# starreeze/drin

Measured on AMD Instinct MI355X. Metric: mention x candidate pairs scored/sec, higher is better.
Workload: dtype bf16x3; 1 GPU; wikimel-shaped scoring forward: 100-cand (+1 answer slot), D=768, R=2048, L=128, P=49, T=64 token-level entity text; parallelism=dp1 (mentions sharded, no collective)

## Files before the change

### drin_amd/csrc/fused.h

```cpp
#pragma once
#include <hip/hip_runtime.h>
#include <stddef.h>
#include <stdint.h>
#include <string.h>

#include "../../include/drin_hip.h"
#include "layout.h"

namespace drin {

struct Prepared {
  size_t wcat1, bcat1, ecat, etmp, k_t, k_i, c_txt, c_img, cb_t, cb_i, total;
  size_t p_ctxt, p_cimg, p_wh2;
  size_t p_wmt, p_wmi, p_wcat1, p_ecat, p_wet, p_wei, p_wh1;
  size_t p_cimg_f16;
  size_t cimg_f16_scale;
  void build(const drin_config& c) {
    const size_t D = c.embed_dim, R = c.image_dim;
    size_t off = 0;
    auto take = [&off](size_t n) {
      const size_t o = off;
      off += (n + 63) & ~(size_t)63;
      return o;
    };
    wcat1 = take(2 * D * D);
    bcat1 = take(2 * D);
    ecat = take(D * (D + R));
    etmp = take(D * (D + R));
    k_t = take(D);
    k_i = take(D);
    c_txt = take(D * D);
    c_img = take(D * R);
    cb_t = take(D);
    cb_i = take(D);
    p_ctxt = take(D * D);
    p_cimg = take(D * R);
    p_wh2 = take(D * D);
    p_wmt = take(D * D);
    p_wmi = take(D * R);
    p_wcat1 = take(2 * D * D);
    p_ecat = take(D * (D + R));
    p_wet = take(D * D);
    p_wei = take(D * R);
    p_wh1 = take(D * D);
    p_cimg_f16 = take(D * R / 2 + 2);
    cimg_f16_scale = take(2);
    total = off;
  }
};

int fused_supported(const drin_config* c);
int cached_chunks_per_mention(const drin_config& c);

struct StreamArgs {
  const void* entity_text;
  const int64_t* entity_mask;
  const void* entity_image;
  const void* entity_object;
  const float* entity_object_score;
  const int64_t* entity_index;
  int64_t num_entities;
  int32_t* index_status;
  const float* miet;
  const float* mtei;
  const float* span_mean;
  const void* mobj;
  const float* mscore;
  const float* fu;
  const float* q;
  const float* k_t;
  const float* k_i;
  float* xt_out;
  void* xt_hi;
  void* xt_lo;
  void* xi_hi;
  void* xi_lo;
  float* xi_scale;
  void* xi_f16;
  float* e0m;
  float* e1m;
  float* s_part;
  float* s_text;
  float* s_img;
  float* sig;
  int B, N, D4, R4, T, Km, Ke, chunks, ldq, ldfu, dynamic, bf16_features;
  int act_e;
  float mask[4];
  float cos_eps, miei_eps, clip;
};

struct PairArgs {
  const float* h_text;
  const float* h_image;
  const float* hm;
  const float* c_t;
  const float* c_i;
  const float* gamma;
  const float* beta;
  const float* e0m;
  const float* e1m;
  float* et1;
  void* et1_hi;
  void* et1_lo;
  float* s2_part;
  int B, N, D4, chunks, ldhm;
  int act_v;
  float ln_eps;
};

struct FinalArgs {
  const float* h2;
  const float* hm2;
  const float* b_h2;
  const float* gamma;
  const float* beta;
  const float* e1m;
  const float* mt2;
  float* scores;
  int B, N, D4, chunks;
  int act_v;
  float ln_eps, cos_eps;
};

template <class Args>
Args shaped_args(const drin_config& c) {
  Args a;
  memset(&a, 0, sizeof(a));
  a.B = c.batch, a.N = c.num_candidates, a.D4 = c.embed_dim / 4;
  return a;
}
template <class Args>
void set_vertex_fields(Args& a, const drin_config& c) {
  a.ln_eps = c.layer_norm_eps, a.act_v = vertex_act(&c);
}
template <class Args>
void set_edge_fields(Args& a, const drin_config& c) {
  a.R4 = c.image_dim / 4;
  a.Km = c.mention_objects;
  a.dynamic = c.dynamic_edges != 0;
  a.act_e = edge_act(&c);
  for (int k = 0; k < 4; ++k) a.mask[k] = c.edge_enabled[k];
  a.cos_eps = c.cosine_eps, a.miei_eps = c.miei_eps, a.clip = c.clip_scale;
}

size_t entity_stream_lds_bytes(const StreamArgs& a);
int launch_entity_stream(const StreamArgs& a, hipStream_t st);
int launch_reduce_stream_partials(const float* part, float* s_text, float* s_img, float* sig, int B, int D, int R,
                                  int chunks, hipStream_t st);
int launch_mention_input1(const float* T, const float* T2, const float* sig, const float* b_et, const float* b_ei,
                          const float* v0, float* out, int B, int D, int N, hipStream_t st);
int launch_pair_layer1(const PairArgs& a, hipStream_t st);
int launch_mention_input2(const float* part, const float* mt1, float* out, int B, int D, int N, int chunks,
                          hipStream_t st);
int launch_pair_final(const FinalArgs& a, hipStream_t st);

struct GemmScratch {
  float* p = nullptr;
  size_t floats = 0;
};
int run_folded_head(const drin_config* cfg, const drin_batch* b, const drin_params* params, const float* prepared, const Prepared& P,
                    bool weight_planes, float* span_mean, float* mimg, float* vm0, float* hmfu, GemmScratch mention_sk, hipStream_t st);
int run_folded_mention_finish(const drin_config* cfg, const drin_params* params, const float* prepared, const Prepared& P,
                              bool weight_planes, float* vm1, float* hm2, GemmScratch mention_sk, hipStream_t st);
int run_folded_tail(const drin_config* cfg, const drin_params* params, const float* prepared, const Prepared& P, int chunks,
                    const float* s2_part, const float* vm1, float* agg2, float* mt2, const float* hm2, const float* e1m, float* h2,
                    const float* et1, const void* et1_hi, bool weight_planes, GemmScratch mention_sk, GemmScratch pair_sk,
                    float* scores, hipStream_t st);
}
```

### drin_amd/csrc/fused_forward.hip

```cpp
#include <string.h>

#include "fused.h"
#include "internal.h"
#include "layout.h"

namespace drin {

constexpr int kMixedMinCandidates = 64;

struct FusedLayout {
  size_t span_mean, mimg, vm0, hmfu, q, e0m, e1m, xt, s_part, s_text, s_img, sig, tm, tm2, agg1, vm1, hm2, h_text, h_image,
      et1, s2_part, agg2, mt2, p_xt, p_xi, p_et1, xi_scale, splitk, splitk_floats, pair_splitk, pair_splitk_floats, total;
  int chunks;
  void build(const drin_config& c) {
    const size_t B = c.batch, N = c.num_candidates, D = c.embed_dim, R = c.image_dim, M = B * N;
    chunks = (int)(B >= 2048 ? (N + 127) / 128 : B >= 1024 ? (N + 47) / 48 : (N + 15) / 16);
    size_t off = 0;
    auto take = [&off](size_t n) {
      const size_t o = off;
      off += (n + 63) & ~(size_t)63;
      return o;
    };
    span_mean = take(B * D);
    mimg = take(B * R);
    vm0 = take(2 * B * D);
    hmfu = take(2 * B * 2 * D);
    q = take(2 * B * (D + R));
    e0m = take(4 * M);
    e1m = take(4 * M);
    xt = take(c.entity_tokens > 0 ? M * D : 0);
    s_part = take(B * chunks * (2 * D + 2 * R + 4));
    s_text = take(2 * B * D);
    s_img = take(2 * B * R);
    sig = take(4 * B);
    tm = take(2 * B * D);
    tm2 = take(2 * B * D);
    agg1 = take(2 * B * D);
    vm1 = take(2 * B * D);
    hm2 = take(2 * B * D);
    h_text = take(M * D);
    h_image = take(M * D);
    et1 = take(M * D);
    s2_part = take(B * chunks * 2 * D);
    agg2 = take(B * D);
    mt2 = take(B * D);
    const bool planes = c.precision == DRIN_PREC_BF16X3 || c.precision == DRIN_PREC_BF16X3_ALL || c.precision == DRIN_PREC_BF16X3_IF16;
    p_xt = take(planes ? M * D : 0);
    p_xi = take(!planes ? 0 : c.num_entities > 0 ? M * R : c.precision == DRIN_PREC_BF16X3_IF16 ? M * R / 2 : 0);
    p_et1 = take(planes ? M * D : 0);
    xi_scale = take(c.precision == DRIN_PREC_BF16X3_IF16 ? M : 0);
    splitk_floats = 2 * B <= 512 ? 8 * 2 * B * (D + R) : 0;
    if (planes && splitk_floats < (size_t)192 * 65536) splitk_floats = (size_t)192 * 65536;
    splitk = take(splitk_floats);
    pair_splitk_floats = 0;
    {
      const size_t tiles = ((M + 255) / 256) * ((D + 255) / 256);
      if (planes && tiles <= 128)
        for (size_t s : {16, 8, 6, 4, 3, 2})
          if (tiles * s <= 256) {
            pair_splitk_floats = s * ((M + 255) / 256 * 256) * D;
            break;
          }
    }
    pair_splitk = take(pair_splitk_floats);
    total = off;
  }
};

static bool if16_gate(const drin_config* c, bool indexed) {
  const int64_t M = (int64_t)c->batch * c->num_candidates;
  return c->precision == DRIN_PREC_BF16X3_IF16 && !indexed && c->feature_dtype == DRIN_FEAT_F32 &&
         c->num_candidates >= kMixedMinCandidates && c->embed_dim == 768 && c->image_dim == 2048 &&
         cdiv(M, 256) * cdiv(c->embed_dim, 256) >= 128;
}

#ifndef DRIN_SIDE_WGS
#define DRIN_SIDE_WGS 64
#endif
#ifndef DRIN_SIDE_PERMILLE
#define DRIN_SIDE_PERMILLE 900
#endif
#ifndef DRIN_SIDE_MIN_TILES
#define DRIN_SIDE_MIN_TILES 1200
#endif
constexpr int kSideWgs = DRIN_SIDE_WGS;
constexpr int kSidePermille = DRIN_SIDE_PERMILLE;
constexpr int64_t kSideMinTiles = DRIN_SIDE_MIN_TILES;
#ifdef DRIN_SIDE_PROBE
static int g_probe_wgs = kSideWgs, g_probe_permille = kSidePermille;
extern "C" __attribute__((visibility("default"))) void drin_probe_side_plan(int wgs, int permille) { g_probe_wgs = wgs, g_probe_permille = permille; }
#endif
struct SidePlan {
  int64_t S = 0;
  int G = 0;
};
static SidePlan image_side_plan(const drin_config* c, bool indexed, bool capturing) {
  SidePlan plan;
  int wgs = kSideWgs, permille = kSidePermille;
#ifdef DRIN_SIDE_PROBE
  wgs = g_probe_wgs, permille = g_probe_permille;
#endif
  const bool split = c->precision == DRIN_PREC_BF16X3 || c->precision == DRIN_PREC_BF16X3_ALL || c->precision == DRIN_PREC_BF16X3_IF16;
  if (capturing || indexed || !split || if16_gate(c, indexed) || wgs <= 0 || permille <= 0) return plan;
  const int D = c->embed_dim, R = c->image_dim;
  if ((D % 32) || (R % 32) || c->batch <= 0) return plan;
  const int64_t M = (int64_t)c->batch * c->num_candidates;
  const int64_t nx = cdiv(D, 256), row_tiles = cdiv(M, 256), tiles = row_tiles * nx;
  if (tiles < 192 || tiles < kSideMinTiles || tiles > ((int64_t)1 << 28)) return plan;
  FusedLayout L;
  L.build(*c);
  const int64_t whole_rows = gemm_p4_whole_tiles(tiles, R, L.splitk_floats > 0, L.splitk_floats) / nx;
  int64_t S = (row_tiles * permille + 500) / 1000;
  S = S < whole_rows ? S : whole_rows;
  S = S < row_tiles - 1 ? S : row_tiles - 1;
  if (S <= 0) return plan;
  plan.S = S;
  plan.G = (int)(wgs < S * nx ? wgs : S * nx);
  return plan;
}

struct SideJoin {
  SideLane* lane = nullptr;
  hipStream_t st = nullptr;
  int join() {
    if (!lane) return DRIN_OK;
    const hipError_t e = hipStreamWaitEvent(st, lane->join, 0);
    lane = nullptr;
    return e == hipSuccess ? DRIN_OK : hip_fail(e, "hipStreamWaitEvent(side stream)");
  }
  ~SideJoin() { (void)join(); }
};

int fused_supported(const drin_config* c) {
  if (c->num_layers != 2) {
    set_error("fused path: built for num_layers == 2 (got %d); use drin_forward", c->num_layers);
    return DRIN_E_UNSUPPORTED;
  }
  if (c->vector_edges) {
    set_error("fused path: vector edge features (model.py:112-116) run on the layer-by-layer path; use drin_forward");
    return DRIN_E_UNSUPPORTED;
  }
  if (c->mention_object_inner > 1 || c->entity_object_inner > 1 || c->entity_image_inner > 1) {
    set_error("fused path: inner feature dims > 1 need the pooled path of drin_forward");
    return DRIN_E_UNSUPPORTED;
  }
  const bool tiny = c->embed_dim <= 256 && c->image_dim <= 256;
  const bool full = c->embed_dim <= 768 && c->image_dim <= 2048;
  if (!tiny && !full) {
    set_error("fused path: D=%d R=%d outside the built instantiations", c->embed_dim, c->image_dim);
    return DRIN_E_UNSUPPORTED;
  }
  return DRIN_OK;
}

}

using namespace drin;

extern "C" {

int drin_split_planes(const float* x, void* hi, void* lo, int64_t n, void* stream) {
  DRIN_BIND_DEVICE(stream, x, "drin_split_planes");
  if (!x || !hi || !lo) {
    set_error("drin_split_planes: NULL argument");
    return DRIN_E_NULL;
  }
  return launch_split_planes(x, hi, lo, n, (hipStream_t)stream);
}

int drin_linear_planes_fwd(const void* x_hi, const void* x_lo, const void* w_hi, const void* w_lo, const float* bias,
                           float* y, int64_t rows, int32_t n_out, int32_t k, void* stream) {
  DRIN_BIND_DEVICE(stream, y, "drin_linear_planes_fwd");
  if (!x_hi || !w_hi || !w_lo || !y) {
    set_error("drin_linear_planes_fwd: NULL argument");
    return DRIN_E_NULL;
  }
  return launch_gemm_x3_planes(x_hi, x_lo, k, w_hi, w_lo, k, bias, y, n_out, rows, n_out, k, (hipStream_t)stream);
}

int drin_fused_supported(const drin_config* cfg) {
  DRIN_TRY(validate_config(cfg));
  return fused_supported(cfg);
}

size_t drin_prepared_bytes(const drin_config* cfg) {
  if (validate_config(cfg) != DRIN_OK || fused_supported(cfg) != DRIN_OK) return 0;
  Prepared P;
  P.build(*cfg);
  return P.total * sizeof(float);
}

int drin_prepare(const drin_config* cfg, const drin_params* params, void* prepared, size_t prepared_bytes,
                 void* stream) {
  DRIN_BIND_DEVICE(stream, prepared, "drin_prepare");
  RoctxRange range("drin_prepare");
  DRIN_TRY(validate_config(cfg));
  DRIN_TRY(fused_supported(cfg));
  if (!params || !prepared) {
    set_error("drin_prepare: NULL argument");
    return DRIN_E_NULL;
  }
  Prepared P;
  P.build(*cfg);
  if (prepared_bytes < P.total * sizeof(float) || !aligned16(prepared)) {
    set_error("drin_prepare: buffer has %zu bytes (needs %zu) or is not 16-byte aligned", prepared_bytes,
              P.total * sizeof(float));
    return DRIN_E_WORKSPACE;
  }
  hipStream_t st = (hipStream_t)stream;
  float* pb = (float*)prepared;
  const int D = cfg->embed_dim, R = cfg->image_dim;
  const drin_layer_params& L1 = params->layer[0];
  const int F32 = DRIN_PREC_F32;
  auto copy = [&](float* dst, const float* src, size_t n) -> int {
    hipError_t e = hipMemcpyAsync(dst, src, n * sizeof(float), hipMemcpyDeviceToDevice, st);
    return e == hipSuccess ? DRIN_OK : hip_fail(e, "hipMemcpyAsync(prepare)");
  };
  DRIN_TRY(copy(pb + P.wcat1, L1.w_h, (size_t)D * D));
  DRIN_TRY(copy(pb + P.wcat1 + (size_t)D * D, L1.w_u, (size_t)D * D));
  {
    hipError_t e = hipMemsetAsync(pb + P.bcat1, 0, D * sizeof(float), st);
    if (e != hipSuccess) return hip_fail(e, "hipMemsetAsync(prepare)");
  }
  DRIN_TRY(copy(pb + P.bcat1 + D, L1.b_u, D));
  DRIN_TRY(launch_gemm_nn(L1.w_v, D, params->w_entity_text, D, pb + P.etmp, D + R, D, D, D, false, F32, st));
  DRIN_TRY(launch_gemm_nn(L1.w_v, D, params->w_entity_image, R, pb + P.etmp + D, D + R, D, R, D, false, F32, st));
  DRIN_TRY(launch_transpose(pb + P.etmp, pb + P.ecat, D, D + R, st));
  DRIN_TRY(launch_gemm_nt(params->b_entity_text, D, L1.w_v, D, L1.b_v, pb + P.k_t, D, 1, D, D, false, F32, st));
  DRIN_TRY(launch_gemm_nt(params->b_entity_image, D, L1.w_v, D, L1.b_v, pb + P.k_i, D, 1, D, D, false, F32, st));
  DRIN_TRY(launch_gemm_nn(L1.w_h, D, params->w_entity_text, D, pb + P.c_txt, D, D, D, D, false, F32, st));
  DRIN_TRY(launch_gemm_nn(L1.w_h, D, params->w_entity_image, R, pb + P.c_img, R, D, R, D, false, F32, st));
  DRIN_TRY(launch_gemm_nt(params->b_entity_text, D, L1.w_h, D, L1.b_h, pb + P.cb_t, D, 1, D, D, false, F32, st));
  DRIN_TRY(launch_gemm_nt(params->b_entity_image, D, L1.w_h, D, L1.b_h, pb + P.cb_i, D, 1, D, D, false, F32, st));
  {
    const size_t dd = (size_t)D * D, dr = (size_t)D * R;
    __bf16* q = reinterpret_cast<__bf16*>(pb + P.p_ctxt);
    DRIN_TRY(launch_split_planes(pb + P.c_txt, q, q + dd, dd, st));
    q = reinterpret_cast<__bf16*>(pb + P.p_cimg);
    DRIN_TRY(launch_split_planes(pb + P.c_img, q, q + dr, dr, st));
    DRIN_TRY(launch_to_f16_scaled(pb + P.c_img, pb + P.p_cimg_f16, (int64_t)dr, pb + P.cimg_f16_scale, st));
    q = reinterpret_cast<__bf16*>(pb + P.p_wh2);
    DRIN_TRY(launch_split_planes(params->layer[1].w_h, q, q + dd, dd, st));
    struct { size_t off; const float* w; size_t n; } extra[] = {
        {P.p_wmt, params->w_mention_text, dd},  {P.p_wmi, params->w_mention_image, dr},
        {P.p_wcat1, pb + P.wcat1, 2 * dd},      {P.p_ecat, pb + P.ecat, dd + dr},
        {P.p_wet, params->w_entity_text, dd},   {P.p_wei, params->w_entity_image, dr},
        {P.p_wh1, L1.w_h, dd}};
    for (const auto& e : extra) {
      q = reinterpret_cast<__bf16*>(pb + e.off);
      DRIN_TRY(launch_split_planes(e.w, q, q + e.n, e.n, st));
    }
  }
  return DRIN_OK;
}

}

namespace drin {

static int folded_precision(const drin_config* c) { return c->precision == DRIN_PREC_BF16X3_IF16 ? (int)DRIN_PREC_BF16X3 : c->precision; }

int run_folded_head(const drin_config* cfg, const drin_batch* b, const drin_params* params, const float* pb, const Prepared& P,
                    bool weight_planes, float* span_mean, float* mimg, float* vm0, float* hmfu, GemmScratch sk, hipStream_t st) {
  const int B = cfg->batch, D = cfg->embed_dim, R = cfg->image_dim, prec = folded_precision(cfg);
  auto wp = [&](size_t plane_off) -> const float* { return weight_planes ? pb + plane_off : nullptr; };
  if (cfg->feature_dtype == DRIN_FEAT_BF16) {
    DRIN_TRY(launch_span_mean_bf16(b->mention_text, b->mention_start, b->mention_end, span_mean, B, cfg->mention_tokens, D, st));
    DRIN_TRY(launch_axis_mean_bf16(b->mention_image, mimg, B, cfg->image_regions, R, st));
  } else {
    DRIN_TRY(launch_span_mean(b->mention_text, b->mention_start, b->mention_end, span_mean, B, cfg->mention_tokens, D, st));
    DRIN_TRY(launch_axis_mean(b->mention_image, mimg, B, cfg->image_regions, R, st));
  }
  DRIN_TRY(launch_gemm_nt_pair({span_mean, params->w_mention_text, params->b_mention_text, vm0, D, D, D, B, D, D, wp(P.p_wmt)},
                               {mimg, params->w_mention_image, params->b_mention_image, vm0 + (size_t)B * D, R, R, D, B, D, R, wp(P.p_wmi)},
                               prec, st, sk.p, sk.floats));
  return launch_gemm_nt(vm0, D, pb + P.wcat1, D, pb + P.bcat1, hmfu, 2 * D, 2 * (int64_t)B, 2 * D, D, false, prec, st, sk.p, sk.floats,
                        wp(P.p_wcat1));
}

int run_folded_mention_finish(const drin_config* cfg, const drin_params* params, const float* pb, const Prepared& P,
                              bool weight_planes, float* vm1, float* hm2, GemmScratch sk, hipStream_t st) {
  const int B = cfg->batch, D = cfg->embed_dim;
  const drin_layer_params& L1 = params->layer[0];
  DRIN_TRY(launch_layernorm_gelu(vm1, L1.ln_weight, L1.ln_bias, vm1, nullptr, nullptr, 2 * (int64_t)B, D, cfg->layer_norm_eps, st,
                                 vertex_act(cfg)));
  return launch_gemm_nt(vm1, D, params->layer[1].w_h, D, nullptr, hm2, D, 2 * (int64_t)B, D, D, false, folded_precision(cfg), st, sk.p,
                        sk.floats, weight_planes ? pb + P.p_wh2 : nullptr);
}

int run_folded_tail(const drin_config* cfg, const drin_params* params, const float* pb, const Prepared& P, int chunks,
                    const float* s2_part, const float* vm1, float* agg2, float* mt2, const float* hm2, const float* e1m, float* h2,
                    const float* et1, const void* et1_hi, bool weight_planes, GemmScratch sk, GemmScratch pair_sk, float* scores,
                    hipStream_t st) {
  const int B = cfg->batch, N = cfg->num_candidates, D = cfg->embed_dim, prec = folded_precision(cfg);
  const int64_t M = (int64_t)B * N;
  const drin_layer_params& L2 = params->layer[1];
  DRIN_TRY(launch_mention_input2(s2_part, vm1, agg2, B, D, N, chunks, st));
  DRIN_TRY(launch_gemm_nt(agg2, D, L2.w_h, D, L2.b_h, mt2, D, B, D, D, false, prec, st, sk.p, sk.floats,
                          weight_planes ? pb + P.p_wh2 : nullptr));
  DRIN_TRY(launch_layernorm_gelu(mt2, L2.ln_weight, L2.ln_bias, mt2, nullptr, nullptr, B, D, cfg->layer_norm_eps, st, vertex_act(cfg)));
  if (et1_hi) {
    const __bf16* e1 = static_cast<const __bf16*>(et1_hi);
    const __bf16* w2 = reinterpret_cast<const __bf16*>(pb + P.p_wh2);
    DRIN_TRY(launch_gemm_x3_planes(e1, e1 + (size_t)M * D, D, w2, w2 + (size_t)D * D, D, nullptr, h2, D, M, D, D, st, pair_sk.p,
                                   pair_sk.floats));
  } else {
    DRIN_TRY(launch_gemm_nt(et1, D, L2.w_h, D, nullptr, h2, D, M, D, D, false, prec, st));
  }
  FinalArgs fa = shaped_args<FinalArgs>(*cfg);
  set_vertex_fields(fa, *cfg);
  fa.h2 = h2;
  fa.hm2 = hm2;
  fa.b_h2 = L2.b_h;
  fa.gamma = L2.ln_weight;
  fa.beta = L2.ln_bias;
  fa.e1m = e1m;
  fa.mt2 = mt2;
  fa.scores = scores;
  fa.chunks = chunks;
  fa.cos_eps = cfg->cosine_eps;
  return launch_pair_final(fa, st);
}

static int forward_prepared_on_stream(const drin_config* cfg, const drin_batch* b, const drin_params* params, const void* prepared,
                                      void* workspace, float* scores, hipStream_t st) {
  FusedLayout L;
  L.build(*cfg);
  Prepared P;
  P.build(*cfg);
  float* ws = (float*)workspace;
  const float* pb = (const float*)prepared;
  const int B = cfg->batch, N = cfg->num_candidates, D = cfg->embed_dim, R = cfg->image_dim;
  const int64_t M = (int64_t)B * N;
  if (B == 0) return DRIN_OK;
  const int prec = folded_precision(cfg);
  const bool dyn = cfg->dynamic_edges != 0;
  const bool tokens = cfg->entity_tokens > 0;
  const bool planes = (prec == DRIN_PREC_BF16X3 || prec == DRIN_PREC_BF16X3_ALL) && (D % 32 == 0) && (R % 32 == 0);
  const bool indexed = b->entity_index != nullptr;
  const bool xi_planes = planes && indexed;
  const bool if16 = if16_gate(cfg, indexed) && gemm_f16_planes_fits(ws + L.p_xi, R, pb + P.p_cimg_f16, R, ws + L.h_image, D, M, D, R);
  hipStreamCaptureStatus capture = hipStreamCaptureStatusNone;
  if (hipStreamIsCapturing(st, &capture) != hipSuccess) {
    (void)hipGetLastError();
    capture = hipStreamCaptureStatusActive;
  }
  SidePlan side = image_side_plan(cfg, indexed, capture != hipStreamCaptureStatusNone);
  if (!aligned16(b->entity_image) || !aligned16(ws + L.h_image) || !b->entity_image) side = SidePlan();
  if (b->entity_text_cls) {
    set_error("drin_forward_prepared: entity_text_cls (text pooled ahead of time) is a form of the training entry points");
    return DRIN_E_UNSUPPORTED;
  }
  if (indexed && cfg->num_entities <= 0) {
    set_error("drin_forward_prepared: entity_index given but cfg.num_entities = %d", cfg->num_entities);
    return DRIN_E_SHAPE;
  }
  if (indexed && !planes) {
    set_error("drin_forward_prepared: entity_index needs the split-bf16 precision (the stream kernel gathers the "
              "GEMM operands as planes); gather on the caller side for DRIN_PREC_F32");
    return DRIN_E_UNSUPPORTED;
  }
  const bool bf16_feat = cfg->feature_dtype == DRIN_FEAT_BF16;
  if (bf16_feat && !planes) {
    set_error("drin_forward_prepared: bf16 features need the split-bf16 precision (DRIN_PREC_BF16X3) and D, R multiples of 32");
    return DRIN_E_UNSUPPORTED;
  }
  __bf16* xt_hi = reinterpret_cast<__bf16*>(ws + L.p_xt);
  __bf16* xi_hi = reinterpret_cast<__bf16*>(ws + L.p_xi);
  __bf16* e1_hi = reinterpret_cast<__bf16*>(ws + L.p_et1);
  const size_t MD = (size_t)M * D, MR = (size_t)M * R;
  const drin_layer_params& L1 = params->layer[0];

  auto wp = [&](size_t plane_off) -> const float* { return planes ? pb + plane_off : nullptr; };
  const GemmScratch msk{L.splitk_floats ? ws + L.splitk : nullptr, L.splitk_floats};
  float* vm0 = ws + L.vm0;
  float* hmfu = ws + L.hmfu;
  const bool xt_exact = bf16_feat && !tokens;
  const GemmScratch psk = L.pair_splitk_floats ? GemmScratch{ws + L.pair_splitk, L.pair_splitk_floats} : msk;
  auto image_rows_product = [&](hipStream_t on, RowTiles rows) -> int {
    const __bf16* ci = reinterpret_cast<const __bf16*>(pb + P.p_cimg);
    if (bf16_feat)
      return launch_gemm_x3_planes(b->entity_image, nullptr, R, ci, ci + (size_t)D * R, R, nullptr, ws + L.h_image, D, M, D, R, on, psk.p,
                                   psk.floats, rows);
    return launch_gemm_nt_bf16x3_p4((const float*)b->entity_image, R, ci, ci + (size_t)D * R, R, nullptr, ws + L.h_image, D, M, D, R, on, false,
                                    aligned16(psk.p) ? psk.p : nullptr, psk.floats, rows);
  };
  SideJoin side_join;
  if (side.S > 0) {
    SideLane* lane = nullptr;
    DRIN_TRY(side_lane(&lane));
    std::lock_guard<std::mutex> order(lane->order);
    hipError_t e = hipEventRecord(lane->fork, st);
    if (e == hipSuccess) e = hipStreamWaitEvent(lane->stream, lane->fork, 0);
    if (e != hipSuccess) return hip_fail(e, "fork to the side stream");
    const int rc = image_rows_product(lane->stream, RowTiles{0, side.S, side.G});
    e = hipEventRecord(lane->join, lane->stream);
    side_join.lane = lane, side_join.st = st;
    if (rc != DRIN_OK) return rc;
    if (e != hipSuccess) return hip_fail(e, "hipEventRecord(side stream)");
  }
  DRIN_TRY(run_folded_head(cfg, b, params, pb, P, planes, ws + L.span_mean, ws + L.mimg, vm0, hmfu, msk, st));
  if (dyn)
    DRIN_TRY(launch_gemm_nt(hmfu + D, 2 * D, pb + P.ecat, D, nullptr, ws + L.q, D + R, 2 * (int64_t)B, D + R, D, false, prec, st, msk.p,
                            msk.floats, wp(P.p_ecat)));
  StreamArgs sa = shaped_args<StreamArgs>(*cfg);
  set_edge_fields(sa, *cfg);
  sa.entity_text = b->entity_text;
  sa.entity_mask = b->entity_text_mask;
  sa.entity_image = b->entity_image;
  sa.entity_object = b->entity_object;
  sa.entity_object_score = b->entity_object_score;
  sa.entity_index = b->entity_index;
  sa.num_entities = cfg->num_entities;
  sa.index_status = b->index_status;
  sa.miet = b->miet_similarity;
  sa.mtei = b->mtei_similarity;
  sa.span_mean = ws + L.span_mean;
  sa.mobj = b->mention_object;
  sa.mscore = b->mention_object_score;
  sa.fu = hmfu + D;
  sa.ldfu = 2 * D;
  sa.q = ws + L.q;
  sa.ldq = D + R;
  sa.k_t = pb + P.k_t;
  sa.k_i = pb + P.k_i;
  sa.xt_out = planes ? nullptr : ws + L.xt;
  if (planes) {
    sa.xt_hi = xt_hi;
    sa.xt_lo = xt_exact ? nullptr : xt_hi + MD;
    if (xi_planes) {
      sa.xi_hi = xi_hi;
      sa.xi_lo = bf16_feat ? nullptr : xi_hi + MR;
    }
  }
  sa.xi_scale = if16 ? ws + L.xi_scale : nullptr;
  sa.xi_f16 = if16 ? static_cast<void*>(xi_hi) : nullptr;
  sa.e0m = ws + L.e0m;
  sa.e1m = ws + L.e1m;
  sa.s_part = ws + L.s_part;
  sa.T = cfg->entity_tokens;
  sa.Ke = cfg->entity_objects;
  sa.chunks = L.chunks;
  sa.bf16_features = bf16_feat ? 1 : 0;
  sa.s_text = ws + L.s_text;
  sa.s_img = ws + L.s_img;
  sa.sig = ws + L.sig;
  DRIN_TRY(launch_entity_stream(sa, st));
  if (L.chunks > 1)
    DRIN_TRY(launch_reduce_stream_partials(ws + L.s_part, ws + L.s_text, ws + L.s_img, ws + L.sig, B, D, R, L.chunks, st));
  DRIN_TRY(launch_gemm_nt_pair({ws + L.s_text, params->w_entity_text, nullptr, ws + L.tm, D, D, D, 2 * (int64_t)B, D, D, wp(P.p_wet)},
                               {ws + L.s_img, params->w_entity_image, nullptr, ws + L.tm2, R, R, D, 2 * (int64_t)B, D, R,
                                wp(P.p_wei)},
                               prec, st, msk.p, msk.floats));
  DRIN_TRY(launch_mention_input1(ws + L.tm, ws + L.tm2, ws + L.sig, params->b_entity_text, params->b_entity_image, vm0, ws + L.agg1, B, D, N, st));
  float* vm1 = ws + L.vm1;
  DRIN_TRY(launch_gemm_nt(ws + L.agg1, D, L1.w_h, D, L1.b_h, vm1, D, 2 * (int64_t)B, D, D, false, prec, st, msk.p, msk.floats, wp(P.p_wh1)));
  DRIN_TRY(run_folded_mention_finish(cfg, params, pb, P, planes, vm1, ws + L.hm2, msk, st));
  if (planes) {
    const __bf16* ct = reinterpret_cast<const __bf16*>(pb + P.p_ctxt);
    const __bf16* ci = reinterpret_cast<const __bf16*>(pb + P.p_cimg);
    DRIN_TRY(launch_gemm_x3_planes(xt_hi, xt_exact ? nullptr : xt_hi + MD, D, ct, ct + (size_t)D * D, D, nullptr, ws + L.h_text, D, M, D,
                                   D, st, psk.p, psk.floats));
    if (if16)
      DRIN_TRY(launch_gemm_f16_planes(xi_hi, R, pb + P.p_cimg_f16, R, ws + L.xi_scale, pb + P.cimg_f16_scale, ws + L.h_image, D, M, D, R,
                                      st, psk.p, psk.floats));
    else if (xi_planes)
      DRIN_TRY(launch_gemm_x3_planes(xi_hi, bf16_feat ? nullptr : xi_hi + MR, R, ci, ci + (size_t)D * R, R, nullptr, ws + L.h_image, D, M,
                                     D, R, st, psk.p, psk.floats));
    else if (side.S > 0) {
      DRIN_TRY(side_join.join());
      DRIN_TRY(image_rows_product(st, RowTiles{side.S, -1, 0}));
    } else if (bf16_feat)
      DRIN_TRY(launch_gemm_x3_planes(b->entity_image, nullptr, R, ci, ci + (size_t)D * R, R, nullptr, ws + L.h_image, D, M, D, R, st, psk.p,
                                     psk.floats));
    else
      DRIN_TRY(launch_gemm_nt_bf16x3(b->entity_image, R, pb + P.c_img, R, nullptr, ws + L.h_image, D, M, D, R, st, ci, ci + (size_t)D * R,
                                     false, psk.p, psk.floats));
  } else {
    const float* x_t = tokens ? ws + L.xt : b->entity_text;
    DRIN_TRY(launch_gemm_nt(x_t, D, pb + P.c_txt, D, nullptr, ws + L.h_text, D, M, D, D, false, prec, st));
    DRIN_TRY(launch_gemm_nt(b->entity_image, R, pb + P.c_img, R, nullptr, ws + L.h_image, D, M, D, R, false, prec, st));
  }
  PairArgs pa = shaped_args<PairArgs>(*cfg);
  set_vertex_fields(pa, *cfg);
  pa.h_text = ws + L.h_text;
  pa.h_image = ws + L.h_image;
  pa.hm = hmfu;
  pa.ldhm = 2 * D;
  pa.c_t = pb + P.cb_t;
  pa.c_i = pb + P.cb_i;
  pa.gamma = L1.ln_weight;
  pa.beta = L1.ln_bias;
  pa.e0m = ws + L.e0m;
  pa.e1m = ws + L.e1m;
  pa.et1 = planes ? nullptr : ws + L.et1;
  if (planes) {
    pa.et1_hi = e1_hi;
    pa.et1_lo = e1_hi + MD;
  }
  pa.s2_part = ws + L.s2_part;
  pa.chunks = L.chunks;
  DRIN_TRY(launch_pair_layer1(pa, st));
  return run_folded_tail(cfg, params, pb, P, L.chunks, ws + L.s2_part, vm1, ws + L.agg2, ws + L.mt2, ws + L.hm2, ws + L.e1m, ws + L.h_text,
                         planes ? nullptr : ws + L.et1, planes ? e1_hi : nullptr, planes, msk, psk, scores, st);
}

}

extern "C" {

int32_t drin_workgroups_per_mention(const drin_config* cfg, int32_t cached) {
  if (validate_config(cfg) != DRIN_OK || fused_supported(cfg) != DRIN_OK) return 0;
  if (cached) return cached_chunks_per_mention(*cfg);
  FusedLayout L;
  L.build(*cfg);
  return L.chunks;
}

int32_t drin_image_contraction_side_tiles(const drin_config* cfg, int32_t indexed) {
  if (validate_config(cfg) != DRIN_OK || fused_supported(cfg) != DRIN_OK) return 0;
  return (int32_t)image_side_plan(cfg, indexed != 0, false).S;
}

int32_t drin_image_contraction_passes(const drin_config* cfg, int32_t indexed) {
  if (validate_config(cfg) != DRIN_OK || fused_supported(cfg) != DRIN_OK) return 0;
  if (cfg->precision == DRIN_PREC_F32) return 0;
  if (if16_gate(cfg, indexed != 0)) return 1;
  return cfg->feature_dtype == DRIN_FEAT_BF16 ? 2 : 3;
}

int drin_index_status(int32_t* index_status, void* stream) {
  if (!index_status) {
    set_error("drin_index_status: NULL argument");
    return DRIN_E_NULL;
  }
  DRIN_BIND_DEVICE(stream, index_status, "drin_index_status");
  int32_t w[4] = {0, 0, 0, 0};
  hipError_t e = hipMemcpyAsync(w, index_status, sizeof(w), hipMemcpyDeviceToHost, (hipStream_t)stream);
  if (e == hipSuccess) e = hipStreamSynchronize((hipStream_t)stream);
  if (e != hipSuccess) return hip_fail(e, "drin_index_status");
  if (w[0] == 0) return DRIN_OK;
  e = hipMemsetAsync(index_status, 0, sizeof(w), (hipStream_t)stream);
  if (e != hipSuccess) return hip_fail(e, "drin_index_status(reset)");
  const long long value = (long long)(((uint64_t)(uint32_t)w[3] << 32) | (uint32_t)w[2]);
  set_error("entity_index out of range: candidate row %lld at pair %d (b * N + n) is outside the entity tables - the row was clamped "
            "and a WRONG entity scored; drin/data.py:87-93 raises IndexError here", value, (int)w[1]);
  return DRIN_E_INDEX;
}

size_t drin_fused_workspace_bytes(const drin_config* cfg) {
  if (validate_config(cfg) != DRIN_OK || fused_supported(cfg) != DRIN_OK) return 0;
  FusedLayout L;
  L.build(*cfg);
  return L.total * sizeof(float);
}

int drin_forward_prepared(const drin_config* cfg, const drin_batch* b, const drin_params* params, const void* prepared,
                          void* workspace, size_t workspace_bytes, float* scores, void* stream) {
  DRIN_BIND_DEVICE(stream, workspace, "drin_forward_prepared");
  RoctxRange range("drin_forward_prepared");
  DRIN_TRY(validate_config(cfg));
  DRIN_TRY(fused_supported(cfg));
  if (!b || !params || !prepared || !workspace || !scores) {
    set_error("drin_forward_prepared: NULL argument");
    return DRIN_E_NULL;
  }
  FusedLayout L;
  L.build(*cfg);
  if (workspace_bytes < L.total * sizeof(float) || !aligned16(workspace)) {
    set_error("drin_forward_prepared: workspace has %zu bytes (needs %zu) or is not 16-byte aligned", workspace_bytes,
              L.total * sizeof(float));
    return DRIN_E_WORKSPACE;
  }
  return forward_prepared_on_stream(cfg, b, params, prepared, workspace, scores, (hipStream_t)stream);
}

}
```

### drin_amd/csrc/fused_kernels.hip

```cpp
#include "device_utils.h"
#include "fused.h"
#include "internal.h"
#include "row_ops.h"

namespace drin {

template <int DV, int RV, bool TOKENS, bool EXACT, typename FT, bool XSCALE = false>
__global__ void __launch_bounds__(256, 2) k_entity_stream(const StreamArgs a) {
  extern __shared__ __attribute__((aligned(16))) float lds[];
  const FT* const f_text = static_cast<const FT*>(a.entity_text);
  const FT* const f_image = static_cast<const FT*>(a.entity_image);
  const FT* const f_object = static_cast<const FT*>(a.entity_object);
  const FT* const f_mobj = static_cast<const FT*>(a.mobj);
  const int D4 = EXACT ? DV * 64 : a.D4, R4 = EXACT ? RV * 64 : a.R4, D = D4 * 4, R = R4 * 4;
  constexpr bool RP = sizeof(FT) == 2 && (RV % 2) == 0;
  auto load_r = [&](const FT* row) -> Row<RV> {
    if constexpr (RP)
      return load_row_stream_pair<RV>(row, (int)(threadIdx.x & 63), R4);
    else
      return load_row_stream<RV>(row, (int)(threadIdx.x & 63), R4);
  };
  float* l_mobj = lds;
  float* l_q = l_mobj + a.Km * R;
  float* l_red = l_q + 2 * R;
  float* l_mt = l_red + 2 * D + 2 * R;
  float* l_small = l_mt + 3 * D;
  const int wave = threadIdx.x >> 6, lane = threadIdx.x & 63;
  const int64_t b = blockIdx.y;
  const int per = (a.N + a.chunks - 1) / a.chunks;
  const int n_begin = blockIdx.x * per, n_end = min(a.N, n_begin + per);
  const bool dyn = a.dynamic != 0;

  for (int i = threadIdx.x; i < a.Km * R4; i += 256) st4(l_mobj + i * 4, ld4(f_mobj + (b * a.Km) * R + i * 4));
  for (int i = threadIdx.x; i < D4; i += 256) st4(l_mt + i * 4, ld4(a.span_mean + b * D + i * 4));
  if (dyn) {
    for (int i = threadIdx.x; i < 2 * R4; i += 256) {
      const int which = i / R4, c4 = i - which * R4;
      st4(l_q + i * 4, ld4(a.q + ((int64_t)which * a.B + b) * a.ldq + D + c4 * 4));
    }
    for (int i = threadIdx.x; i < 2 * D4; i += 256) {
      const int which = i / D4, c4 = i - which * D4;
      st4(l_mt + D + i * 4, ld4(a.q + ((int64_t)which * a.B + b) * a.ldq + c4 * 4));
    }
  }
  __syncthreads();
  for (int i = wave; i < a.Km; i += 4) {
    float s = 0.f;
    for (int c4 = lane; c4 < R4; c4 += 64) {
      const float4 v = ld4(l_mobj + i * R + c4 * 4);
      s += dot4(v, v);
    }
    s = wave_sum(s);
    if (lane == 0) l_small[i] = fmaxf(sqrtf(s), a.cos_eps);
  }
  float m_t_norm;
  {
    const Row<DV> m_t = load_row<DV>(l_mt, lane, D4);
    m_t_norm = fmaxf(sqrtf(wave_sum(dot_rows<DV>(m_t, m_t))), a.cos_eps);
  }
  float kap_tt = 0.f, kap_ti = 0.f, kap_it = 0.f, kap_ii = 0.f;
  if (dyn) {
    const Row<DV> fu_t = load_row<DV>(a.fu + b * a.ldfu, lane, D4);
    const Row<DV> fu_i = load_row<DV>(a.fu + ((int64_t)a.B + b) * a.ldfu, lane, D4);
    const Row<DV> k_t = load_row<DV>(a.k_t, lane, D4), k_i = load_row<DV>(a.k_i, lane, D4);
    kap_tt = wave_sum(dot_rows<DV>(fu_t, k_t));
    kap_ti = wave_sum(dot_rows<DV>(fu_t, k_i));
    kap_it = wave_sum(dot_rows<DV>(fu_i, k_t));
    kap_ii = wave_sum(dot_rows<DV>(fu_i, k_i));
  }
  __syncthreads();

  Row<DV> S_tt = zero_row<DV>(), S_it = zero_row<DV>();
  Row<RV> S_ti = zero_row<RV>(), S_ii = zero_row<RV>();
  float sg_tt = 0.f, sg_ti = 0.f, sg_it = 0.f, sg_ii = 0.f;
  const float inv_d = 1.0f / (float)D;

  for (int n = n_begin + wave; n < n_end; n += 4) {
    const int64_t p = b * a.N + n;
    int64_t e = p;
    if (a.entity_index) {
      const int64_t raw = a.entity_index[p];
      e = raw < 0 ? 0 : (raw >= a.num_entities ? a.num_entities - 1 : raw);
      if (e != raw && lane == 0) report_bad_index(a.index_status, p, raw);
    }
    Row<DV> xt;
    float tt;
    if (TOKENS) {
      const int T = a.T;
      int cnt = 0;
      for (int t = lane; t < T; t += 64) cnt += (int)a.entity_mask[e * T + t];
      cnt = (int)wave_sum((float)cnt);
      int stop = cnt - 1;
      if (stop < 0) stop += T;
      stop = stop < 0 ? 0 : (stop > T ? T : stop);
      const FT* base = f_text + e * (int64_t)T * D;
      constexpr bool FLAT = sizeof(FT) == 2 && EXACT && DV == 3;
      const Row<DV> cls = load_row_stream<DV>(base, lane, D4);
      Row<DV> acc = zero_row<DV>();
      int t = 1;
      if constexpr (FLAT) {
        float f0[8], f1[8], f2[8];
#pragma unroll
        for (int i = 0; i < 8; ++i) f0[i] = f1[i] = f2[i] = 0.f;
        const char* flat = reinterpret_cast<const char*>(base) + (size_t)lane * 16;
        auto add8 = [](float (&f)[8], const u32x4_t v) {
#pragma unroll
          for (int i = 0; i < 4; ++i) {
            f[2 * i] += __builtin_bit_cast(float, v[i] << 16);
            f[2 * i + 1] += __builtin_bit_cast(float, v[i] & 0xffff0000u);
          }
        };
        for (; t + 8 <= stop; t += 8) {
          u32x4_t r[4][3];
#pragma unroll
          for (int u = 0; u < 4; ++u)
#pragma unroll
            for (int k = 0; k < 3; ++k) r[u][k] = ld16_stream(flat + (size_t)(t + 2 * u) * (2 * 768) + k * 1024);
#pragma unroll
          for (int u = 0; u < 4; ++u) {
            add8(f0, r[u][0]);
            add8(f1, r[u][1]);
            add8(f2, r[u][2]);
          }
        }
        for (; t + 2 <= stop; t += 2) {
          const u32x4_t r0 = ld16_stream(flat + (size_t)t * (2 * 768)), r1 = ld16_stream(flat + (size_t)t * (2 * 768) + 1024),
                        r2 = ld16_stream(flat + (size_t)t * (2 * 768) + 2048);
          add8(f0, r0);
          add8(f1, r1);
          add8(f2, r2);
        }
        float* scr = l_red + wave * 768;
#pragma unroll
        for (int i = 0; i < 8; ++i) {
          const float y1 = __shfl_xor(f1[i], 32), y2 = __shfl_xor(f2[i], 32);
          f0[i] += lane < 32 ? y1 : y2;
          f1[i] += y2;
        }
        st4(scr + 8 * lane, make_float4(f0[0], f0[1], f0[2], f0[3]));
        st4(scr + 8 * lane + 4, make_float4(f0[4], f0[5], f0[6], f0[7]));
        if (lane < 32) {
          st4(scr + 512 + 8 * lane, make_float4(f1[0], f1[1], f1[2], f1[3]));
          st4(scr + 512 + 8 * lane + 4, make_float4(f1[4], f1[5], f1[6], f1[7]));
        }
        __builtin_amdgcn_wave_barrier();
#pragma unroll
        for (int j = 0; j < DV; ++j) acc.v[j] = ld4(scr + 4 * (lane + 64 * j));
        __builtin_amdgcn_wave_barrier();
      } else if constexpr (sizeof(FT) == 2 && (EXACT || DV == 1)) {
        for (; t + 8 <= stop; t += 8) {
          Row<DV> r[8];
#pragma unroll
          for (int u = 0; u < 8; ++u) r[u] = load_row_stream<DV>(base + (int64_t)(t + u) * D, lane, D4);
#pragma unroll
          for (int u = 0; u < 8; ++u)
#pragma unroll
            for (int j = 0; j < DV; ++j) acc.v[j] = acc.v[j] + r[u].v[j];
        }
      }
      for (; t + 4 <= stop; t += 4) {
        const Row<DV> r0 = load_row_stream<DV>(base + (int64_t)t * D, lane, D4);
        const Row<DV> r1 = load_row_stream<DV>(base + (int64_t)(t + 1) * D, lane, D4);
        const Row<DV> r2 = load_row_stream<DV>(base + (int64_t)(t + 2) * D, lane, D4);
        const Row<DV> r3 = load_row_stream<DV>(base + (int64_t)(t + 3) * D, lane, D4);
#pragma unroll
        for (int j = 0; j < DV; ++j) acc.v[j] = (((acc.v[j] + r0.v[j]) + r1.v[j]) + r2.v[j]) + r3.v[j];
      }
      for (; t < stop; ++t) {
        const Row<DV> r0 = load_row_stream<DV>(base + (int64_t)t * D, lane, D4);
#pragma unroll
        for (int j = 0; j < DV; ++j) acc.v[j] = acc.v[j] + r0.v[j];
      }
      const float den = stop > 1 ? (float)(stop - 1) : 0.0f;
#pragma unroll
      for (int j = 0; j < DV; ++j)
        xt.v[j] = make_float4(acc.v[j].x / den, acc.v[j].y / den, acc.v[j].z / den, acc.v[j].w / den);
      if (a.xt_out) store_row<DV>(a.xt_out + p * D, xt, lane, D4);
      const float xy = wave_sum(dot_row_lds<DV>(cls, l_mt, lane, D4)), yy = wave_sum(dot_rows<DV>(cls, cls));
      tt = xy / (m_t_norm * fmaxf(sqrtf(yy), a.cos_eps));
    } else {
      xt = load_row_stream<DV>(f_text + e * D, lane, D4);
      const float xy = wave_sum(dot_row_lds<DV>(xt, l_mt, lane, D4)), yy = wave_sum(dot_rows<DV>(xt, xt));
      tt = xy / (m_t_norm * fmaxf(sqrtf(yy), a.cos_eps));
    }
    if (a.xt_hi) store_row_planes<DV>(a.xt_hi, a.xt_lo, p * D, xt, lane, D4);
    float sim = 0.f, wsum = 0.f;
    for (int j = 0; j < a.Ke; ++j) {
      const Row<RV> eo = load_r(f_object + (e * a.Ke + j) * R);
      const float ny = fmaxf(sqrtf(wave_sum(dot_rows<RV>(eo, eo))), a.cos_eps);
      const float es = a.entity_object_score[e * a.Ke + j];
      for (int i = 0; i < a.Km; ++i) {
        const float xy = wave_sum(dot_row_lds<RV, RP>(eo, l_mobj + i * R, lane, R4));
        const float w = a.mscore[b * a.Km + i] * es;
        sim += xy / (l_small[i] * ny) * w;
        wsum += w;
      }
    }
    const float ii = sim / (wsum + a.miei_eps);
    const Row<RV> xi = load_r(f_image + e * R);
    if (a.xi_hi) store_row_planes<RV, RP>(a.xi_hi, a.xi_lo, p * R, xi, lane, R4);
    if constexpr (XSCALE) {
      float m = 0.f;
#pragma unroll
      for (int j = 0; j < RV; ++j) m = fmaxf(m, fmaxf(fmaxf(fabsf(xi.v[j].x), fabsf(xi.v[j].y)), fmaxf(fabsf(xi.v[j].z), fabsf(xi.v[j].w))));
      const float sc = cache_field_scale(wave_max(m));
      if (lane == 0) a.xi_scale[p] = sc;
      store_row_f16_scaled<RV, RP>(a.xi_f16, p * R, xi, 1.0f / sc, lane);
    }
    const float e_tt = tt * a.mask[0];
    const float e_ti = (a.mtei[p] / a.clip) * a.mask[1];
    const float e_it = (a.miet[p] / a.clip) * a.mask[2];
    const float e_ii = ii * a.mask[3];
    float n_tt = e_tt, n_ti = e_ti, n_it = e_it, n_ii = e_ii;
    if (dyn) {
      const float d_tt = wave_sum(dot_row_lds<DV>(xt, l_mt + D, lane, D4));
      const float d_it = wave_sum(dot_row_lds<DV>(xt, l_mt + 2 * D, lane, D4));
      const float d_ti = wave_sum(dot_row_lds<RV, RP>(xi, l_q, lane, R4));
      const float d_ii = wave_sum(dot_row_lds<RV, RP>(xi, l_q + R, lane, R4));
      n_tt = edge_act_apply(a.act_e, (d_tt + kap_tt) * inv_d + e_tt);
      n_ti = edge_act_apply(a.act_e, (d_ti + kap_ti) * inv_d + e_ti);
      n_it = edge_act_apply(a.act_e, (d_it + kap_it) * inv_d + e_it);
      n_ii = edge_act_apply(a.act_e, (d_ii + kap_ii) * inv_d + e_ii);
    }
    if (lane == 0) {
      const int64_t M = (int64_t)a.B * a.N;
      a.e0m[p] = e_tt;
      a.e0m[M + p] = e_ti;
      a.e0m[2 * M + p] = e_it;
      a.e0m[3 * M + p] = e_ii;
      a.e1m[p] = n_tt * a.mask[0];
      a.e1m[M + p] = n_ti * a.mask[1];
      a.e1m[2 * M + p] = n_it * a.mask[2];
      a.e1m[3 * M + p] = n_ii * a.mask[3];
    }
    axpy_row<DV>(S_tt, e_tt, xt);
    axpy_row<DV>(S_it, e_it, xt);
    axpy_row<RV>(S_ti, e_ti, xi);
    axpy_row<RV>(S_ii, e_ii, xi);
    sg_tt += e_tt;
    sg_ti += e_ti;
    sg_it += e_it;
    sg_ii += e_ii;
  }

  for (int w = 0; w < 4; ++w) {
    __syncthreads();
    if (wave == w) {
#pragma unroll
      for (int j = 0; j < DV; ++j) {
        const int c4 = lane + 64 * j;
        if (c4 < D4) {
          float* p0 = l_red + c4 * 4;
          float* p1 = l_red + D + c4 * 4;
          st4(p0, w == 0 ? S_tt.v[j] : ld4(p0) + S_tt.v[j]);
          st4(p1, w == 0 ? S_it.v[j] : ld4(p1) + S_it.v[j]);
        }
      }
#pragma unroll
      for (int j = 0; j < RV; ++j) {
        const int c4 = row_col4<RP>(lane, j);
        if (c4 < R4) {
          float* p0 = l_red + 2 * D + c4 * 4;
          float* p1 = l_red + 2 * D + R + c4 * 4;
          st4(p0, w == 0 ? S_ti.v[j] : ld4(p0) + S_ti.v[j]);
          st4(p1, w == 0 ? S_ii.v[j] : ld4(p1) + S_ii.v[j]);
        }
      }
      if (lane == 0) {
        float* s4 = l_small + a.Km;
        s4[0] = (w == 0 ? 0.f : s4[0]) + sg_tt;
        s4[1] = (w == 0 ? 0.f : s4[1]) + sg_ti;
        s4[2] = (w == 0 ? 0.f : s4[2]) + sg_it;
        s4[3] = (w == 0 ? 0.f : s4[3]) + sg_ii;
      }
    }
  }
  __syncthreads();
  if (a.chunks == 1) {
    for (int i = threadIdx.x; i < 2 * D4; i += 256) {
      const int which = i / D4, c4 = i - which * D4;
      st4(a.s_text + ((int64_t)which * a.B + b) * D + c4 * 4, ld4(l_red + i * 4));
    }
    for (int i = threadIdx.x; i < 2 * R4; i += 256) {
      const int which = i / R4, c4 = i - which * R4;
      st4(a.s_img + ((int64_t)which * a.B + b) * R + c4 * 4, ld4(l_red + 2 * D + i * 4));
    }
    if (threadIdx.x < 4) a.sig[(int64_t)threadIdx.x * a.B + b] = l_small[a.Km + threadIdx.x];
    return;
  }
  float* out = a.s_part + (b * a.chunks + blockIdx.x) * (int64_t)(2 * D + 2 * R + 4);
  for (int i = threadIdx.x; i < (2 * D + 2 * R) / 4; i += 256) st4(out + i * 4, ld4(l_red + i * 4));
  if (threadIdx.x < 4) out[2 * D + 2 * R + threadIdx.x] = l_small[a.Km + threadIdx.x];
}

size_t entity_stream_lds_bytes(const StreamArgs& a) {
  const size_t D = (size_t)a.D4 * 4, R = (size_t)a.R4 * 4;
  return sizeof(float) * (a.Km * R + 2 * R + 2 * D + 2 * R + 3 * D + a.Km + 4);
}

template <int DV, int RV, bool TOKENS, bool EXACT, typename FT, bool XSCALE = false>
static int launch_stream_ft(const StreamArgs& a, hipStream_t st) {
  const size_t lds = entity_stream_lds_bytes(a);
  auto kern = k_entity_stream<DV, RV, TOKENS, EXACT, FT, XSCALE>;
  static DynLdsOptIn opt_in;
  if (lds > 48 * 1024)
    DRIN_TRY(ensure_dynamic_lds(opt_in, reinterpret_cast<const void*>(kern), (int)lds, "hipFuncSetAttribute(entity_stream)"));
  KernelTimer timer(DRIN_KC_STREAM, st);
  hipLaunchKernelGGL(kern, dim3((unsigned)a.chunks, (unsigned)a.B), dim3(256), lds, st, a);
  DRIN_CHECK_LAUNCH("k_entity_stream");
  return DRIN_OK;
}

template <int DV, int RV, bool TOKENS, bool EXACT>
static int launch_stream_t(const StreamArgs& a, hipStream_t st) {
  if (a.xi_scale != nullptr) {
    if constexpr (EXACT && DV == 3) {
      if (a.xi_f16 == nullptr) {
        set_error("entity_stream: xi_scale without xi_f16");
        return DRIN_E_NULL;
      }
      if (!a.bf16_features) return launch_stream_ft<DV, RV, TOKENS, EXACT, float, true>(a, st);
    }
    set_error("entity_stream: the scaled fp16 image plane is built for fp32-stored rows at D = 768, R = 2048");
    return DRIN_E_UNSUPPORTED;
  }
  return a.bf16_features ? launch_stream_ft<DV, RV, TOKENS, EXACT, __bf16>(a, st)
                         : launch_stream_ft<DV, RV, TOKENS, EXACT, float>(a, st);
}

int launch_entity_stream(const StreamArgs& a, hipStream_t st) {
  if (a.B <= 0) return DRIN_OK;
  if (a.B > 65535) {
    set_error("entity_stream: batch %d exceeds the grid limit; split the batch", a.B);
    return DRIN_E_SHAPE;
  }
  const bool tok = a.T > 0;
  if (a.D4 <= 64 && a.R4 <= 64)
    return tok ? launch_stream_t<1, 1, true, false>(a, st) : launch_stream_t<1, 1, false, false>(a, st);
  if (a.D4 == 192 && a.R4 == 512)
    return tok ? launch_stream_t<3, 8, true, true>(a, st) : launch_stream_t<3, 8, false, true>(a, st);
  if (a.D4 <= 192 && a.R4 <= 512)
    return tok ? launch_stream_t<3, 8, true, false>(a, st) : launch_stream_t<3, 8, false, false>(a, st);
  set_error("entity_stream: D=%d R=%d outside the built instantiations", a.D4 * 4, a.R4 * 4);
  return DRIN_E_UNSUPPORTED;
}

__global__ void __launch_bounds__(256) k_reduce_stream_partials(const float* __restrict__ part, float* __restrict__ s_text,
                                                                float* __restrict__ s_img, float* __restrict__ sig,
                                                                int B, int D, int R, int chunks) {
  const int64_t b = blockIdx.y;
  const int width = 2 * D + 2 * R + 4;
  const int i = (blockIdx.x * 256 + threadIdx.x) * 4;
  if (i >= width) return;
  const float* src = part + (b * chunks) * (int64_t)width + i;
  float4 s = make_float4(0.f, 0.f, 0.f, 0.f);
  int c = 0;
  for (; c + 4 <= chunks; c += 4) {
    const float4 v0 = ld4(src + (int64_t)c * width), v1 = ld4(src + (int64_t)(c + 1) * width);
    const float4 v2 = ld4(src + (int64_t)(c + 2) * width), v3 = ld4(src + (int64_t)(c + 3) * width);
    s = (((s + v0) + v1) + v2) + v3;
  }
  for (; c < chunks; ++c) s = s + ld4(src + (int64_t)c * width);
  if (i < D) {
    st4(s_text + b * D + i, s);
  } else if (i < 2 * D) {
    st4(s_text + ((int64_t)B + b) * D + (i - D), s);
  } else if (i < 2 * D + R) {
    st4(s_img + b * R + (i - 2 * D), s);
  } else if (i < 2 * D + 2 * R) {
    st4(s_img + ((int64_t)B + b) * R + (i - 2 * D - R), s);
  } else {
    sig[b] = s.x;
    sig[(int64_t)B + b] = s.y;
    sig[2 * (int64_t)B + b] = s.z;
    sig[3 * (int64_t)B + b] = s.w;
  }
}

int launch_reduce_stream_partials(const float* part, float* s_text, float* s_img, float* sig, int B, int D, int R,
                                  int chunks, hipStream_t st) {
  if (B <= 0) return DRIN_OK;
  KernelTimer timer(DRIN_KC_GCN, st);
  hipLaunchKernelGGL(k_reduce_stream_partials, dim3((unsigned)cdiv((2 * D + 2 * R + 4) / 4, 256), (unsigned)B), dim3(256), 0,
                     st, part, s_text, s_img, sig, B, D, R, chunks);
  DRIN_CHECK_LAUNCH("k_reduce_stream_partials");
  return DRIN_OK;
}

__global__ void __launch_bounds__(256) k_mention_input1(const float* __restrict__ T, const float* __restrict__ T2,
                                                        const float* __restrict__ sig,
                                                        const float* __restrict__ b_et, const float* __restrict__ b_ei,
                                                        const float* __restrict__ v0, float* __restrict__ out, int B,
                                                        int D, float inv_n) {
  const int64_t i = (int64_t)blockIdx.x * 256 + threadIdx.x;
  if (i >= 2 * (int64_t)B * D) return;
  const int d = (int)(i % D);
  const int64_t row = i / D;
  const int t = (int)(row / B);
  const int64_t b = row - (int64_t)t * B;
  const float sa = sig[(int64_t)(t == 0 ? 0 : 2) * B + b], sb = sig[(int64_t)(t == 0 ? 1 : 3) * B + b];
  out[i] = ((T[i] + T2[i]) + sa * b_et[d] + sb * b_ei[d]) * inv_n + v0[i];
}

int launch_mention_input1(const float* T, const float* T2, const float* sig, const float* b_et, const float* b_ei,
                          const float* v0, float* out, int B, int D, int N, hipStream_t st) {
  if (B <= 0) return DRIN_OK;
  KernelTimer timer(DRIN_KC_GCN, st);
  hipLaunchKernelGGL(k_mention_input1, dim3((unsigned)cdiv(2 * (int64_t)B * D, 256)), dim3(256), 0, st, T, T2, sig,
                     b_et, b_ei, v0, out, B, D, 1.0f / (float)N);
  DRIN_CHECK_LAUNCH("k_mention_input1");
  return DRIN_OK;
}

__global__ void __launch_bounds__(256) k_transpose(const float* __restrict__ in, float* __restrict__ out, int rows,
                                                   int cols) {
  __shared__ float tile[32][33];
  const int tx = threadIdx.x & 31, ty = threadIdx.x >> 5;
  const int r0 = blockIdx.y * 32, c0 = blockIdx.x * 32;
  for (int i = ty; i < 32; i += 8)
    if (r0 + i < rows && c0 + tx < cols) tile[i][tx] = in[(int64_t)(r0 + i) * cols + c0 + tx];
  __syncthreads();
  for (int i = ty; i < 32; i += 8)
    if (c0 + i < cols && r0 + tx < rows) out[(int64_t)(c0 + i) * rows + r0 + tx] = tile[tx][i];
}

int launch_transpose(const float* in, float* out, int rows, int cols, hipStream_t st) {
  if (rows <= 0 || cols <= 0) return DRIN_OK;
  KernelTimer timer(DRIN_KC_GCN, st);
  hipLaunchKernelGGL(k_transpose, dim3((unsigned)cdiv(cols, 32), (unsigned)cdiv(rows, 32)), dim3(256), 0, st, in, out,
                     rows, cols);
  DRIN_CHECK_LAUNCH("k_transpose");
  return DRIN_OK;
}

template <int DV, bool EXACT, bool GENERIC_ACT = false>
__global__ void __launch_bounds__(256) k_pair_layer1(const PairArgs a) {
  __shared__ __attribute__((aligned(16))) float l_red[2 * DV * 256];
  __shared__ __attribute__((aligned(16))) float l_const[6 * DV * 256];
  const int D4 = EXACT ? DV * 64 : a.D4, D = D4 * 4;
  const int wave = threadIdx.x >> 6, lane = threadIdx.x & 63;
  const int64_t b = blockIdx.y;
  const int64_t M = (int64_t)a.B * a.N;
  const int per = (a.N + a.chunks - 1) / a.chunks;
  const int n_begin = blockIdx.x * per, n_end = min(a.N, n_begin + per);
  constexpr int LD = DV * 256;
  {
    const float* src[6] = {a.hm + b * a.ldhm, a.hm + ((int64_t)a.B + b) * a.ldhm, a.c_t, a.c_i, a.gamma, a.beta};
#pragma unroll
    for (int v = 0; v < 6; ++v)
      for (int i = threadIdx.x; i < D4; i += 256) st4(l_const + v * LD + i * 4, ld4(src[v] + i * 4));
  }
  __syncthreads();
  const float *l_hm_t = l_const, *l_hm_i = l_const + LD, *l_ct = l_const + 2 * LD, *l_ci = l_const + 3 * LD;
  const float *l_gamma = l_const + 4 * LD, *l_beta = l_const + 5 * LD;
  Row<DV> S_t = zero_row<DV>(), S_i = zero_row<DV>();
  for (int n = n_begin + wave; n < n_end; n += 4) {
    const int64_t p = b * a.N + n;
    const Row<DV> ht = load_row_stream<DV>(a.h_text + p * D, lane, D4);
    const Row<DV> hi = load_row_stream<DV>(a.h_image + p * D, lane, D4);
    const float e_tt = a.e0m[p], e_ti = a.e0m[M + p], e_it = a.e0m[2 * M + p], e_ii = a.e0m[3 * M + p];
    const Row<DV> et1 = ln_gelu_row_lds<DV, GENERIC_ACT>(combine_rows_lds<DV>(ht, e_tt, l_hm_t, e_it, l_hm_i, l_ct, lane, D4),
                                                         l_gamma, l_beta, lane, D4, a.ln_eps, a.act_v);
    if (a.et1) store_row<DV>(a.et1 + p * D, et1, lane, D4);
    if (a.et1_hi) store_row_planes<DV>(a.et1_hi, a.et1_lo, p * D, et1, lane, D4);
    axpy_row_pk<DV>(S_t, a.e1m[p], et1);
    const Row<DV> ei1 = ln_gelu_row_lds<DV, GENERIC_ACT>(combine_rows_lds<DV>(hi, e_ti, l_hm_t, e_ii, l_hm_i, l_ci, lane, D4),
                                                         l_gamma, l_beta, lane, D4, a.ln_eps, a.act_v);
    axpy_row_pk<DV>(S_i, a.e1m[M + p], ei1);
  }
  for (int w = 0; w < 4; ++w) {
    __syncthreads();
    if (wave == w) {
#pragma unroll
      for (int j = 0; j < DV; ++j) {
        float* p0 = l_red + (j * 64 + lane) * 4;
        float* p1 = l_red + DV * 256 + (j * 64 + lane) * 4;
        st4(p0, w == 0 ? S_t.v[j] : ld4(p0) + S_t.v[j]);
        st4(p1, w == 0 ? S_i.v[j] : ld4(p1) + S_i.v[j]);
      }
    }
  }
  __syncthreads();
  float* out = a.s2_part + (b * a.chunks + blockIdx.x) * (int64_t)(2 * D);
  for (int i = threadIdx.x; i < 2 * D4; i += 256) {
    const int which = i / D4, c4 = i - which * D4;
    st4(out + which * D + c4 * 4, ld4(l_red + which * DV * 256 + c4 * 4));
  }
}

int launch_pair_layer1(const PairArgs& a, hipStream_t st) {
  if (a.B <= 0) return DRIN_OK;
  KernelTimer timer(DRIN_KC_GCN, st);
  if (a.act_v != DRIN_ACT_GELU && a.D4 <= 64)
    hipLaunchKernelGGL((k_pair_layer1<1, false, true>), dim3((unsigned)a.chunks, (unsigned)a.B), dim3(256), 0, st, a);
  else if (a.act_v != DRIN_ACT_GELU && a.D4 <= 192)
    hipLaunchKernelGGL((k_pair_layer1<3, false, true>), dim3((unsigned)a.chunks, (unsigned)a.B), dim3(256), 0, st, a);
  else if (a.D4 <= 64)
    hipLaunchKernelGGL((k_pair_layer1<1, false>), dim3((unsigned)a.chunks, (unsigned)a.B), dim3(256), 0, st, a);
  else if (a.D4 == 192)
    hipLaunchKernelGGL((k_pair_layer1<3, true>), dim3((unsigned)a.chunks, (unsigned)a.B), dim3(256), 0, st, a);
  else if (a.D4 < 192)
    hipLaunchKernelGGL((k_pair_layer1<3, false>), dim3((unsigned)a.chunks, (unsigned)a.B), dim3(256), 0, st, a);
  else {
    set_error("pair_layer1: D=%d outside the built instantiations", a.D4 * 4);
    return DRIN_E_UNSUPPORTED;
  }
  DRIN_CHECK_LAUNCH("k_pair_layer1");
  return DRIN_OK;
}

__global__ void __launch_bounds__(256) k_mention_input2(const float* __restrict__ part, const float* __restrict__ mt1,
                                                        float* __restrict__ out, int D, int chunks, float inv_n) {
  const int64_t b = blockIdx.y;
  const int d = blockIdx.x * 256 + threadIdx.x;
  if (d >= D) return;
  float st = 0.f, si = 0.f;
  for (int c = 0; c < chunks; ++c) {
    const float* p = part + (b * chunks + c) * (int64_t)(2 * D);
    st += p[d];
    si += p[D + d];
  }
  out[b * D + d] = (st * inv_n + si * inv_n) + mt1[b * D + d];
}

int launch_mention_input2(const float* part, const float* mt1, float* out, int B, int D, int N, int chunks,
                          hipStream_t st) {
  if (B <= 0) return DRIN_OK;
  KernelTimer timer(DRIN_KC_GCN, st);
  hipLaunchKernelGGL(k_mention_input2, dim3((unsigned)cdiv(D, 256), (unsigned)B), dim3(256), 0, st, part, mt1, out, D,
                     chunks, 1.0f / (float)N);
  DRIN_CHECK_LAUNCH("k_mention_input2");
  return DRIN_OK;
}

template <int DV, bool EXACT, bool GENERIC_ACT = false>
__global__ void __launch_bounds__(256) k_pair_final(const FinalArgs a) {
  __shared__ __attribute__((aligned(16))) float l_const[6 * DV * 256];
  const int D4 = EXACT ? DV * 64 : a.D4, D = D4 * 4;
  const int wave = threadIdx.x >> 6, lane = threadIdx.x & 63;
  const int64_t b = blockIdx.y;
  const int64_t M = (int64_t)a.B * a.N;
  const int per = (a.N + a.chunks - 1) / a.chunks;
  const int n_begin = blockIdx.x * per, n_end = min(a.N, n_begin + per);
  constexpr int LD = DV * 256;
  {
    const float* src[6] = {a.hm2 + b * D, a.hm2 + ((int64_t)a.B + b) * D, a.b_h2, a.gamma, a.beta, a.mt2 + b * D};
#pragma unroll
    for (int v = 0; v < 6; ++v)
      for (int i = threadIdx.x; i < D4; i += 256) st4(l_const + v * LD + i * 4, ld4(src[v] + i * 4));
  }
  __syncthreads();
  const Row<DV> mt2 = load_row<DV>(l_const + 5 * LD, lane, D4);
  const float xx = wave_sum(dot_rows<DV>(mt2, mt2));
  for (int n = n_begin + wave; n < n_end; n += 4) {
    const int64_t p = b * a.N + n;
    const Row<DV> h = load_row_stream<DV>(a.h2 + p * D, lane, D4);
    const Row<DV> et2 = ln_gelu_row_lds<DV, GENERIC_ACT>(
        combine_rows_lds<DV>(h, a.e1m[p], l_const, a.e1m[2 * M + p], l_const + LD, l_const + 2 * LD, lane, D4),
        l_const + 3 * LD, l_const + 4 * LD, lane, D4, a.ln_eps, a.act_v);
    const float xy = wave_sum(dot_rows_pk<DV>(mt2, et2));
    const float yy = wave_sum(dot_rows_pk<DV>(et2, et2));
    if (lane == 0) a.scores[p] = cosine_from_sums(xy, xx, yy, a.cos_eps);
  }
}

int launch_pair_final(const FinalArgs& a, hipStream_t st) {
  if (a.B <= 0) return DRIN_OK;
  KernelTimer timer(DRIN_KC_GCN, st);
  if (a.act_v != DRIN_ACT_GELU && a.D4 <= 64)
    hipLaunchKernelGGL((k_pair_final<1, false, true>), dim3((unsigned)a.chunks, (unsigned)a.B), dim3(256), 0, st, a);
  else if (a.act_v != DRIN_ACT_GELU && a.D4 <= 192)
    hipLaunchKernelGGL((k_pair_final<3, false, true>), dim3((unsigned)a.chunks, (unsigned)a.B), dim3(256), 0, st, a);
  else if (a.D4 <= 64)
    hipLaunchKernelGGL((k_pair_final<1, false>), dim3((unsigned)a.chunks, (unsigned)a.B), dim3(256), 0, st, a);
  else if (a.D4 == 192)
    hipLaunchKernelGGL((k_pair_final<3, true>), dim3((unsigned)a.chunks, (unsigned)a.B), dim3(256), 0, st, a);
  else if (a.D4 < 192)
    hipLaunchKernelGGL((k_pair_final<3, false>), dim3((unsigned)a.chunks, (unsigned)a.B), dim3(256), 0, st, a);
  else {
    set_error("pair_final: D=%d outside the built instantiations", a.D4 * 4);
    return DRIN_E_UNSUPPORTED;
  }
  DRIN_CHECK_LAUNCH("k_pair_final");
  return DRIN_OK;
}

}
```

Baseline: 28.34 million pairs/s.

## Fold mention layer-1 aggregation into pair kernel using precomputed h_text/h_image sums

Rather than have the entity stream kernel accumulate edge-weighted entity text/image sums and then run two GEMMs (through the entity projections and layer-1 weights), the pair layer-1 kernel now accumulates edge-weighted sums of the already-projected h_text/h_image rows plus edge-weight totals. A new small kernel combines them with precomputed bias-projected vectors to produce vm1 directly. This drops the large image-dim reductions from the stream kernel, two GEMMs, and several weight plane copies, and shrinks stream LDS use. It also raises occupancy bounds on the stream and pair kernels, widens the stream unroll, disables the side-GEMM overlap when LDS allows co-residency, and tweaks the side permille. The pair kernel takes on more register and LDS pressure, and the IF16 path still needs an image-sum reduction and GEMM.

```diff
diff --git a/drin_amd/csrc/fused.h b/drin_amd/csrc/fused.h
--- a/drin_amd/csrc/fused.h
+++ b/drin_amd/csrc/fused.h
@@ -10,9 +10,9 @@
 namespace drin {
 
 struct Prepared {
-  size_t wcat1, bcat1, ecat, etmp, k_t, k_i, c_txt, c_img, cb_t, cb_i, total;
+  size_t wcat1, bcat1, ecat, etmp, k_t, k_i, c_txt, c_img, cb_t, cb_i, hb_t, hb_i, total;
   size_t p_ctxt, p_cimg, p_wh2;
-  size_t p_wmt, p_wmi, p_wcat1, p_ecat, p_wet, p_wei, p_wh1;
+  size_t p_wmt, p_wmi, p_wcat1, p_ecat;
   size_t p_cimg_f16;
   size_t cimg_f16_scale;
   void build(const drin_config& c) {
@@ -40,11 +40,10 @@
     p_wmi = take(D * R);
     p_wcat1 = take(2 * D * D);
     p_ecat = take(D * (D + R));
-    p_wet = take(D * D);
-    p_wei = take(D * R);
-    p_wh1 = take(D * D);
     p_cimg_f16 = take(D * R / 2 + 2);
     cimg_f16_scale = take(2);
+    hb_t = take(D);
+    hb_i = take(D);
     total = off;
   }
 };
@@ -79,10 +78,7 @@
   void* xi_f16;
   float* e0m;
   float* e1m;
-  float* s_part;
-  float* s_text;
-  float* s_img;
-  float* sig;
+  float* simg_part;
   int B, N, D4, R4, T, Km, Ke, chunks, ldq, ldfu, dynamic, bf16_features;
   int act_e;
   float mask[4];
@@ -103,7 +99,9 @@
   void* et1_hi;
   void* et1_lo;
   float* s2_part;
+  float* s1_part;
   int B, N, D4, chunks, ldhm;
+  int u_text_only;
   int act_v;
   float ln_eps;
 };
@@ -145,11 +143,10 @@
 
 size_t entity_stream_lds_bytes(const StreamArgs& a);
 int launch_entity_stream(const StreamArgs& a, hipStream_t st);
-int launch_reduce_stream_partials(const float* part, float* s_text, float* s_img, float* sig, int B, int D, int R,
-                                  int chunks, hipStream_t st);
-int launch_mention_input1(const float* T, const float* T2, const float* sig, const float* b_et, const float* b_ei,
-                          const float* v0, float* out, int B, int D, int N, hipStream_t st);
 int launch_pair_layer1(const PairArgs& a, hipStream_t st);
+int launch_mention_layer1(const float* part, const float* hb_t, const float* hb_i, const float* hm, int ldhm, const float* b_h1,
+                          const float* u_img, float* out, int B, int D, int N, int chunks, hipStream_t st);
+int launch_sum_image_partials(const float* part, float* s_img, int B, int R, int chunks, hipStream_t st);
 int launch_mention_input2(const float* part, const float* mt1, float* out, int B, int D, int N, int chunks,
                           hipStream_t st);
 int launch_pair_final(const FinalArgs& a, hipStream_t st);
diff --git a/drin_amd/csrc/fused_forward.hip b/drin_amd/csrc/fused_forward.hip
--- a/drin_amd/csrc/fused_forward.hip
+++ b/drin_amd/csrc/fused_forward.hip
@@ -9,7 +9,7 @@
 constexpr int kMixedMinCandidates = 64;
 
 struct FusedLayout {
-  size_t span_mean, mimg, vm0, hmfu, q, e0m, e1m, xt, s_part, s_text, s_img, sig, tm, tm2, agg1, vm1, hm2, h_text, h_image,
+  size_t span_mean, mimg, vm0, hmfu, q, e0m, e1m, xt, s1_part, simg_part, s_img, u_img, vm1, hm2, h_text, h_image,
       et1, s2_part, agg2, mt2, p_xt, p_xi, p_et1, xi_scale, splitk, splitk_floats, pair_splitk, pair_splitk_floats, total;
   int chunks;
   void build(const drin_config& c) {
@@ -29,13 +29,11 @@
     e0m = take(4 * M);
     e1m = take(4 * M);
     xt = take(c.entity_tokens > 0 ? M * D : 0);
-    s_part = take(B * chunks * (2 * D + 2 * R + 4));
-    s_text = take(2 * B * D);
-    s_img = take(2 * B * R);
-    sig = take(4 * B);
-    tm = take(2 * B * D);
-    tm2 = take(2 * B * D);
-    agg1 = take(2 * B * D);
+    s1_part = take(B * chunks * (2 * D + 4));
+    const bool if16_sums = c.precision == DRIN_PREC_BF16X3_IF16;
+    simg_part = take(if16_sums ? B * chunks * 2 * R : 0);
+    s_img = take(if16_sums ? 2 * B * R : 0);
+    u_img = take(if16_sums ? 2 * B * D : 0);
     vm1 = take(2 * B * D);
     hm2 = take(2 * B * D);
     h_text = take(M * D);
@@ -78,7 +76,7 @@
 #define DRIN_SIDE_WGS 64
 #endif
 #ifndef DRIN_SIDE_PERMILLE
-#define DRIN_SIDE_PERMILLE 900
+#define DRIN_SIDE_PERMILLE 850
 #endif
 #ifndef DRIN_SIDE_MIN_TILES
 #define DRIN_SIDE_MIN_TILES 1200
@@ -90,6 +88,14 @@
 static int g_probe_wgs = kSideWgs, g_probe_permille = kSidePermille;
 extern "C" __attribute__((visibility("default"))) void drin_probe_side_plan(int wgs, int permille) { g_probe_wgs = wgs, g_probe_permille = permille; }
 #endif
+constexpr size_t kCuLdsBytes = 160 * 1024, kSideGemmLdsBytes = 128 * 1024;
+static bool stream_shares_cu_with_side_gemm(const drin_config& c) {
+  StreamArgs sa = shaped_args<StreamArgs>(c);
+  set_edge_fields(sa, c);
+  sa.T = c.entity_tokens;
+  sa.bf16_features = c.feature_dtype == DRIN_FEAT_BF16;
+  return entity_stream_lds_bytes(sa) + kSideGemmLdsBytes <= kCuLdsBytes;
+}
 struct SidePlan {
   int64_t S = 0;
   int G = 0;
@@ -104,6 +110,7 @@
   if (capturing || indexed || !split || if16_gate(c, indexed) || wgs <= 0 || permille <= 0) return plan;
   const int D = c->embed_dim, R = c->image_dim;
   if ((D % 32) || (R % 32) || c->batch <= 0) return plan;
+  if (stream_shares_cu_with_side_gemm(*c)) return plan;
   const int64_t M = (int64_t)c->batch * c->num_candidates;
   const int64_t nx = cdiv(D, 256), row_tiles = cdiv(M, 256), tiles = row_tiles * nx;
   if (tiles < 192 || tiles < kSideMinTiles || tiles > ((int64_t)1 << 28)) return plan;
@@ -232,6 +239,8 @@
   DRIN_TRY(launch_gemm_nn(L1.w_h, D, params->w_entity_image, R, pb + P.c_img, R, D, R, D, false, F32, st));
   DRIN_TRY(launch_gemm_nt(params->b_entity_text, D, L1.w_h, D, L1.b_h, pb + P.cb_t, D, 1, D, D, false, F32, st));
   DRIN_TRY(launch_gemm_nt(params->b_entity_image, D, L1.w_h, D, L1.b_h, pb + P.cb_i, D, 1, D, D, false, F32, st));
+  DRIN_TRY(launch_gemm_nt(params->b_entity_text, D, L1.w_h, D, nullptr, pb + P.hb_t, D, 1, D, D, false, F32, st));
+  DRIN_TRY(launch_gemm_nt(params->b_entity_image, D, L1.w_h, D, nullptr, pb + P.hb_i, D, 1, D, D, false, F32, st));
   {
     const size_t dd = (size_t)D * D, dr = (size_t)D * R;
     __bf16* q = reinterpret_cast<__bf16*>(pb + P.p_ctxt);
@@ -243,9 +252,7 @@
     DRIN_TRY(launch_split_planes(params->layer[1].w_h, q, q + dd, dd, st));
     struct { size_t off; const float* w; size_t n; } extra[] = {
         {P.p_wmt, params->w_mention_text, dd},  {P.p_wmi, params->w_mention_image, dr},
-        {P.p_wcat1, pb + P.wcat1, 2 * dd},      {P.p_ecat, pb + P.ecat, dd + dr},
-        {P.p_wet, params->w_entity_text, dd},   {P.p_wei, params->w_entity_image, dr},
-        {P.p_wh1, L1.w_h, dd}};
+        {P.p_wcat1, pb + P.wcat1, 2 * dd},      {P.p_ecat, pb + P.ecat, dd + dr}};
     for (const auto& e : extra) {
       q = reinterpret_cast<__bf16*>(pb + e.off);
       DRIN_TRY(launch_split_planes(e.w, q, q + e.n, e.n, st));
@@ -435,27 +442,14 @@
   }
   sa.xi_scale = if16 ? ws + L.xi_scale : nullptr;
   sa.xi_f16 = if16 ? static_cast<void*>(xi_hi) : nullptr;
+  sa.simg_part = if16 ? ws + L.simg_part : nullptr;
   sa.e0m = ws + L.e0m;
   sa.e1m = ws + L.e1m;
-  sa.s_part = ws + L.s_part;
   sa.T = cfg->entity_tokens;
   sa.Ke = cfg->entity_objects;
   sa.chunks = L.chunks;
   sa.bf16_features = bf16_feat ? 1 : 0;
-  sa.s_text = ws + L.s_text;
-  sa.s_img = ws + L.s_img;
-  sa.sig = ws + L.sig;
   DRIN_TRY(launch_entity_stream(sa, st));
-  if (L.chunks > 1)
-    DRIN_TRY(launch_reduce_stream_partials(ws + L.s_part, ws + L.s_text, ws + L.s_img, ws + L.sig, B, D, R, L.chunks, st));
-  DRIN_TRY(launch_gemm_nt_pair({ws + L.s_text, params->w_entity_text, nullptr, ws + L.tm, D, D, D, 2 * (int64_t)B, D, D, wp(P.p_wet)},
-                               {ws + L.s_img, params->w_entity_image, nullptr, ws + L.tm2, R, R, D, 2 * (int64_t)B, D, R,
-                                wp(P.p_wei)},
-                               prec, st, msk.p, msk.floats));
-  DRIN_TRY(launch_mention_input1(ws + L.tm, ws + L.tm2, ws + L.sig, params->b_entity_text, params->b_entity_image, vm0, ws + L.agg1, B, D, N, st));
-  float* vm1 = ws + L.vm1;
-  DRIN_TRY(launch_gemm_nt(ws + L.agg1, D, L1.w_h, D, L1.b_h, vm1, D, 2 * (int64_t)B, D, D, false, prec, st, msk.p, msk.floats, wp(P.p_wh1)));
-  DRIN_TRY(run_folded_mention_finish(cfg, params, pb, P, planes, vm1, ws + L.hm2, msk, st));
   if (planes) {
     const __bf16* ct = reinterpret_cast<const __bf16*>(pb + P.p_ctxt);
     const __bf16* ci = reinterpret_cast<const __bf16*>(pb + P.p_cimg);
@@ -499,8 +493,19 @@
     pa.et1_lo = e1_hi + MD;
   }
   pa.s2_part = ws + L.s2_part;
+  pa.s1_part = ws + L.s1_part;
+  pa.u_text_only = if16 ? 1 : 0;
   pa.chunks = L.chunks;
   DRIN_TRY(launch_pair_layer1(pa, st));
+  float* vm1 = ws + L.vm1;
+  if (if16) {
+    DRIN_TRY(launch_sum_image_partials(ws + L.simg_part, ws + L.s_img, B, R, L.chunks, st));
+    DRIN_TRY(launch_gemm_nt(ws + L.s_img, R, pb + P.c_img, R, nullptr, ws + L.u_img, D, 2 * (int64_t)B, D, R, false, prec, st, msk.p,
+                            msk.floats, wp(P.p_cimg)));
+  }
+  DRIN_TRY(launch_mention_layer1(ws + L.s1_part, pb + P.hb_t, pb + P.hb_i, hmfu, 2 * D, L1.b_h, if16 ? ws + L.u_img : nullptr, vm1, B, D,
+                                 N, L.chunks, st));
+  DRIN_TRY(run_folded_mention_finish(cfg, params, pb, P, planes, vm1, ws + L.hm2, msk, st));
   return run_folded_tail(cfg, params, pb, P, L.chunks, ws + L.s2_part, vm1, ws + L.agg2, ws + L.mt2, ws + L.hm2, ws + L.e1m, ws + L.h_text,
                          planes ? nullptr : ws + L.et1, planes ? e1_hi : nullptr, planes, msk, psk, scores, st);
 }
diff --git a/drin_amd/csrc/fused_kernels.hip b/drin_amd/csrc/fused_kernels.hip
--- a/drin_amd/csrc/fused_kernels.hip
+++ b/drin_amd/csrc/fused_kernels.hip
@@ -5,8 +5,20 @@
 
 namespace drin {
 
+#ifndef DRIN_STREAM_WAVES
+#define DRIN_STREAM_WAVES 3
+#endif
+#ifndef DRIN_STREAM_ROWS
+#define DRIN_STREAM_ROWS 4
+#endif
+template <typename FT, bool XSCALE>
+constexpr int stream_waves_per_simd() {
+  return sizeof(FT) == 4 && !XSCALE ? DRIN_STREAM_WAVES : 2;
+}
+constexpr int kStreamRows = DRIN_STREAM_ROWS;
+
 template <int DV, int RV, bool TOKENS, bool EXACT, typename FT, bool XSCALE = false>
-__global__ void __launch_bounds__(256, 2) k_entity_stream(const StreamArgs a) {
+__global__ void __launch_bounds__(256, (stream_waves_per_simd<FT, XSCALE>())) k_entity_stream(const StreamArgs a) {
   extern __shared__ __attribute__((aligned(16))) float lds[];
   const FT* const f_text = static_cast<const FT*>(a.entity_text);
   const FT* const f_image = static_cast<const FT*>(a.entity_image);
@@ -22,9 +34,11 @@
   };
   float* l_mobj = lds;
   float* l_q = l_mobj + a.Km * R;
-  float* l_red = l_q + 2 * R;
-  float* l_mt = l_red + 2 * D + 2 * R;
-  float* l_small = l_mt + 3 * D;
+  float* l_mt = l_q + 2 * R;
+  constexpr bool FLAT = TOKENS && sizeof(FT) == 2 && EXACT && DV == 3;
+  float* l_scr = l_mt + 3 * D;
+  float* l_red = l_scr + (FLAT ? 4 * 768 : 0);
+  float* l_small = l_red + (XSCALE ? 2 * R : 0);
   const int wave = threadIdx.x >> 6, lane = threadIdx.x & 63;
   const int64_t b = blockIdx.y;
   const int per = (a.N + a.chunks - 1) / a.chunks;
@@ -70,10 +84,8 @@
   }
   __syncthreads();
 
-  Row<DV> S_tt = zero_row<DV>(), S_it = zero_row<DV>();
-  Row<RV> S_ti = zero_row<RV>(), S_ii = zero_row<RV>();
-  float sg_tt = 0.f, sg_ti = 0.f, sg_it = 0.f, sg_ii = 0.f;
   const float inv_d = 1.0f / (float)D;
+  Row<XSCALE ? RV : 1> S_ti = zero_row<XSCALE ? RV : 1>(), S_ii = zero_row<XSCALE ? RV : 1>();
 
   for (int n = n_begin + wave; n < n_end; n += 4) {
     const int64_t p = b * a.N + n;
@@ -94,7 +106,6 @@
       if (stop < 0) stop += T;
       stop = stop < 0 ? 0 : (stop > T ? T : stop);
       const FT* base = f_text + e * (int64_t)T * D;
-      constexpr bool FLAT = sizeof(FT) == 2 && EXACT && DV == 3;
       const Row<DV> cls = load_row_stream<DV>(base, lane, D4);
       Row<DV> acc = zero_row<DV>();
       int t = 1;
@@ -130,7 +141,7 @@
           add8(f1, r1);
           add8(f2, r2);
         }
-        float* scr = l_red + wave * 768;
+        float* scr = l_scr + wave * 768;
 #pragma unroll
         for (int i = 0; i < 8; ++i) {
           const float y1 = __shfl_xor(f1[i], 32), y2 = __shfl_xor(f2[i], 32);
@@ -158,13 +169,17 @@
             for (int j = 0; j < DV; ++j) acc.v[j] = acc.v[j] + r[u].v[j];
         }
       }
-      for (; t + 4 <= stop; t += 4) {
-        const Row<DV> r0 = load_row_stream<DV>(base + (int64_t)t * D, lane, D4);
-        const Row<DV> r1 = load_row_stream<DV>(base + (int64_t)(t + 1) * D, lane, D4);
-        const Row<DV> r2 = load_row_stream<DV>(base + (int64_t)(t + 2) * D, lane, D4);
-        const Row<DV> r3 = load_row_stream<DV>(base + (int64_t)(t + 3) * D, lane, D4);
-#pragma unroll
-        for (int j = 0; j < DV; ++j) acc.v[j] = (((acc.v[j] + r0.v[j]) + r1.v[j]) + r2.v[j]) + r3.v[j];
+      {
+        constexpr int NR = sizeof(FT) == 4 && !XSCALE ? kStreamRows : 4;
+        for (; t + NR <= stop; t += NR) {
+          Row<DV> r[NR];
+#pragma unroll
+          for (int u = 0; u < NR; ++u) r[u] = load_row_stream<DV>(base + (int64_t)(t + u) * D, lane, D4);
+#pragma unroll
+          for (int u = 0; u < NR; ++u)
+#pragma unroll
+            for (int j = 0; j < DV; ++j) acc.v[j] = acc.v[j] + r[u].v[j];
+        }
       }
       for (; t < stop; ++t) {
         const Row<DV> r0 = load_row_stream<DV>(base + (int64_t)t * D, lane, D4);
@@ -233,69 +248,37 @@
       a.e1m[2 * M + p] = n_it * a.mask[2];
       a.e1m[3 * M + p] = n_ii * a.mask[3];
     }
-    axpy_row<DV>(S_tt, e_tt, xt);
-    axpy_row<DV>(S_it, e_it, xt);
-    axpy_row<RV>(S_ti, e_ti, xi);
-    axpy_row<RV>(S_ii, e_ii, xi);
-    sg_tt += e_tt;
-    sg_ti += e_ti;
-    sg_it += e_it;
-    sg_ii += e_ii;
-  }
-
-  for (int w = 0; w < 4; ++w) {
+    if constexpr (XSCALE) {
+      axpy_row<RV>(S_ti, e_ti, xi);
+      axpy_row<RV>(S_ii, e_ii, xi);
+    }
+  }
+  if constexpr (XSCALE) {
+    for (int w = 0; w < 4; ++w) {
+      __syncthreads();
+      if (wave == w) {
+#pragma unroll
+        for (int j = 0; j < RV; ++j) {
+          const int c4 = row_col4<RP>(lane, j);
+          if (c4 < R4) {
+            float* p0 = l_red + c4 * 4;
+            float* p1 = l_red + R + c4 * 4;
+            st4(p0, w == 0 ? S_ti.v[j] : ld4(p0) + S_ti.v[j]);
+            st4(p1, w == 0 ? S_ii.v[j] : ld4(p1) + S_ii.v[j]);
+          }
+        }
+      }
+    }
     __syncthreads();
-    if (wave == w) {
-#pragma unroll
-      for (int j = 0; j < DV; ++j) {
-        const int c4 = lane + 64 * j;
-        if (c4 < D4) {
-          float* p0 = l_red + c4 * 4;
-          float* p1 = l_red + D + c4 * 4;
-          st4(p0, w == 0 ? S_tt.v[j] : ld4(p0) + S_tt.v[j]);
-          st4(p1, w == 0 ? S_it.v[j] : ld4(p1) + S_it.v[j]);
-        }
-      }
-#pragma unroll
-      for (int j = 0; j < RV; ++j) {
-        const int c4 = row_col4<RP>(lane, j);
-        if (c4 < R4) {
-          float* p0 = l_red + 2 * D + c4 * 4;
-          float* p1 = l_red + 2 * D + R + c4 * 4;
-          st4(p0, w == 0 ? S_ti.v[j] : ld4(p0) + S_ti.v[j]);
-          st4(p1, w == 0 ? S_ii.v[j] : ld4(p1) + S_ii.v[j]);
-        }
-      }
-      if (lane == 0) {
-        float* s4 = l_small + a.Km;
-        s4[0] = (w == 0 ? 0.f : s4[0]) + sg_tt;
-        s4[1] = (w == 0 ? 0.f : s4[1]) + sg_ti;
-        s4[2] = (w == 0 ? 0.f : s4[2]) + sg_it;
-        s4[3] = (w == 0 ? 0.f : s4[3]) + sg_ii;
-      }
-    }
-  }
-  __syncthreads();
-  if (a.chunks == 1) {
-    for (int i = threadIdx.x; i < 2 * D4; i += 256) {
-      const int which = i / D4, c4 = i - which * D4;
-      st4(a.s_text + ((int64_t)which * a.B + b) * D + c4 * 4, ld4(l_red + i * 4));
-    }
-    for (int i = threadIdx.x; i < 2 * R4; i += 256) {
-      const int which = i / R4, c4 = i - which * R4;
-      st4(a.s_img + ((int64_t)which * a.B + b) * R + c4 * 4, ld4(l_red + 2 * D + i * 4));
-    }
-    if (threadIdx.x < 4) a.sig[(int64_t)threadIdx.x * a.B + b] = l_small[a.Km + threadIdx.x];
-    return;
-  }
-  float* out = a.s_part + (b * a.chunks + blockIdx.x) * (int64_t)(2 * D + 2 * R + 4);
-  for (int i = threadIdx.x; i < (2 * D + 2 * R) / 4; i += 256) st4(out + i * 4, ld4(l_red + i * 4));
-  if (threadIdx.x < 4) out[2 * D + 2 * R + threadIdx.x] = l_small[a.Km + threadIdx.x];
+    float* out = a.simg_part + (b * a.chunks + blockIdx.x) * (int64_t)(2 * R);
+    for (int i = threadIdx.x; i < 2 * R4; i += 256) st4(out + i * 4, ld4(l_red + i * 4));
+  }
 }
 
 size_t entity_stream_lds_bytes(const StreamArgs& a) {
   const size_t D = (size_t)a.D4 * 4, R = (size_t)a.R4 * 4;
-  return sizeof(float) * (a.Km * R + 2 * R + 2 * D + 2 * R + 3 * D + a.Km + 4);
+  const bool flat = a.bf16_features && a.T > 0 && a.D4 == 192 && a.R4 == 512;
+  return sizeof(float) * (a.Km * R + 2 * R + 3 * D + (flat ? 4 * 768 : 0) + (a.xi_scale ? 2 * R : 0) + a.Km);
 }
 
 template <int DV, int RV, bool TOKENS, bool EXACT, typename FT, bool XSCALE = false>
@@ -315,8 +298,8 @@
 static int launch_stream_t(const StreamArgs& a, hipStream_t st) {
   if (a.xi_scale != nullptr) {
     if constexpr (EXACT && DV == 3) {
-      if (a.xi_f16 == nullptr) {
-        set_error("entity_stream: xi_scale without xi_f16");
+      if (a.xi_f16 == nullptr || a.simg_part == nullptr) {
+        set_error("entity_stream: xi_scale without xi_f16 / simg_part");
         return DRIN_E_NULL;
       }
       if (!a.bf16_features) return launch_stream_ft<DV, RV, TOKENS, EXACT, float, true>(a, st);
@@ -343,73 +326,6 @@
     return tok ? launch_stream_t<3, 8, true, false>(a, st) : launch_stream_t<3, 8, false, false>(a, st);
   set_error("entity_stream: D=%d R=%d outside the built instantiations", a.D4 * 4, a.R4 * 4);
   return DRIN_E_UNSUPPORTED;
-}
-
-__global__ void __launch_bounds__(256) k_reduce_stream_partials(const float* __restrict__ part, float* __restrict__ s_text,
-                                                                float* __restrict__ s_img, float* __restrict__ sig,
-                                                                int B, int D, int R, int chunks) {
-  const int64_t b = blockIdx.y;
-  const int width = 2 * D + 2 * R + 4;
-  const int i = (blockIdx.x * 256 + threadIdx.x) * 4;
-  if (i >= width) return;
-  const float* src = part + (b * chunks) * (int64_t)width + i;
-  float4 s = make_float4(0.f, 0.f, 0.f, 0.f);
-  int c = 0;
-  for (; c + 4 <= chunks; c += 4) {
-    const float4 v0 = ld4(src + (int64_t)c * width), v1 = ld4(src + (int64_t)(c + 1) * width);
-    const float4 v2 = ld4(src + (int64_t)(c + 2) * width), v3 = ld4(src + (int64_t)(c + 3) * width);
-    s = (((s + v0) + v1) + v2) + v3;
-  }
-  for (; c < chunks; ++c) s = s + ld4(src + (int64_t)c * width);
-  if (i < D) {
-    st4(s_text + b * D + i, s);
-  } else if (i < 2 * D) {
-    st4(s_text + ((int64_t)B + b) * D + (i - D), s);
-  } else if (i < 2 * D + R) {
-    st4(s_img + b * R + (i - 2 * D), s);
-  } else if (i < 2 * D + 2 * R) {
-    st4(s_img + ((int64_t)B + b) * R + (i - 2 * D - R), s);
-  } else {
-    sig[b] = s.x;
-    sig[(int64_t)B + b] = s.y;
-    sig[2 * (int64_t)B + b] = s.z;
-    sig[3 * (int64_t)B + b] = s.w;
-  }
-}
-
-int launch_reduce_stream_partials(const float* part, float* s_text, float* s_img, float* sig, int B, int D, int R,
-                                  int chunks, hipStream_t st) {
-  if (B <= 0) return DRIN_OK;
-  KernelTimer timer(DRIN_KC_GCN, st);
-  hipLaunchKernelGGL(k_reduce_stream_partials, dim3((unsigned)cdiv((2 * D + 2 * R + 4) / 4, 256), (unsigned)B), dim3(256), 0,
-                     st, part, s_text, s_img, sig, B, D, R, chunks);
-  DRIN_CHECK_LAUNCH("k_reduce_stream_partials");
-  return DRIN_OK;
-}
-
-__global__ void __launch_bounds__(256) k_mention_input1(const float* __restrict__ T, const float* __restrict__ T2,
-                                                        const float* __restrict__ sig,
-                                                        const float* __restrict__ b_et, const float* __restrict__ b_ei,
-                                                        const float* __restrict__ v0, float* __restrict__ out, int B,
-                                                        int D, float inv_n) {
-  const int64_t i = (int64_t)blockIdx.x * 256 + threadIdx.x;
-  if (i >= 2 * (int64_t)B * D) return;
-  const int d = (int)(i % D);
-  const int64_t row = i / D;
-  const int t = (int)(row / B);
-  const int64_t b = row - (int64_t)t * B;
-  const float sa = sig[(int64_t)(t == 0 ? 0 : 2) * B + b], sb = sig[(int64_t)(t == 0 ? 1 : 3) * B + b];
-  out[i] = ((T[i] + T2[i]) + sa * b_et[d] + sb * b_ei[d]) * inv_n + v0[i];
-}
-
-int launch_mention_input1(const float* T, const float* T2, const float* sig, const float* b_et, const float* b_ei,
-                          const float* v0, float* out, int B, int D, int N, hipStream_t st) {
-  if (B <= 0) return DRIN_OK;
-  KernelTimer timer(DRIN_KC_GCN, st);
-  hipLaunchKernelGGL(k_mention_input1, dim3((unsigned)cdiv(2 * (int64_t)B * D, 256)), dim3(256), 0, st, T, T2, sig,
-                     b_et, b_ei, v0, out, B, D, 1.0f / (float)N);
-  DRIN_CHECK_LAUNCH("k_mention_input1");
-  return DRIN_OK;
 }
 
 __global__ void __launch_bounds__(256) k_transpose(const float* __restrict__ in, float* __restrict__ out, int rows,
@@ -434,8 +350,8 @@
 }
 
 template <int DV, bool EXACT, bool GENERIC_ACT = false>
-__global__ void __launch_bounds__(256) k_pair_layer1(const PairArgs a) {
-  __shared__ __attribute__((aligned(16))) float l_red[2 * DV * 256];
+__global__ void __launch_bounds__(256, 3) k_pair_layer1(const PairArgs a) {
+  __shared__ __attribute__((aligned(16))) float l_red[4 * DV * 256 + 4];
   __shared__ __attribute__((aligned(16))) float l_const[6 * DV * 256];
   const int D4 = EXACT ? DV * 64 : a.D4, D = D4 * 4;
   const int wave = threadIdx.x >> 6, lane = threadIdx.x & 63;
@@ -452,13 +368,26 @@
   }
   __syncthreads();
   const float *l_hm_t = l_const, *l_hm_i = l_const + LD, *l_ct = l_const + 2 * LD, *l_ci = l_const + 3 * LD;
-  const float *l_gamma = l_const + 4 * LD, *l_beta = l_const + 5 * LD;
-  Row<DV> S_t = zero_row<DV>(), S_i = zero_row<DV>();
+  Row<DV> S_t = zero_row<DV>(), S_i = zero_row<DV>(), U_t = zero_row<DV>(), U_i = zero_row<DV>();
+  float sg_tt = 0.f, sg_ti = 0.f, sg_it = 0.f, sg_ii = 0.f;
   for (int n = n_begin + wave; n < n_end; n += 4) {
     const int64_t p = b * a.N + n;
     const Row<DV> ht = load_row_stream<DV>(a.h_text + p * D, lane, D4);
     const Row<DV> hi = load_row_stream<DV>(a.h_image + p * D, lane, D4);
     const float e_tt = a.e0m[p], e_ti = a.e0m[M + p], e_it = a.e0m[2 * M + p], e_ii = a.e0m[3 * M + p];
+    int trip = 0;
+    asm volatile("" : "+v"(trip));
+    const float *l_gamma = l_const + 4 * LD + trip, *l_beta = l_const + 5 * LD + trip;
+    axpy_row_pk<DV>(U_t, e_tt, ht);
+    axpy_row_pk<DV>(U_i, e_it, ht);
+    if (!a.u_text_only) {
+      axpy_row_pk<DV>(U_t, e_ti, hi);
+      axpy_row_pk<DV>(U_i, e_ii, hi);
+    }
+    sg_tt += e_tt;
+    sg_ti += e_ti;
+    sg_it += e_it;
+    sg_ii += e_ii;
     const Row<DV> et1 = ln_gelu_row_lds<DV, GENERIC_ACT>(combine_rows_lds<DV>(ht, e_tt, l_hm_t, e_it, l_hm_i, l_ct, lane, D4),
                                                          l_gamma, l_beta, lane, D4, a.ln_eps, a.act_v);
     if (a.et1) store_row<DV>(a.et1 + p * D, et1, lane, D4);
@@ -474,18 +403,33 @@
 #pragma unroll
       for (int j = 0; j < DV; ++j) {
         float* p0 = l_red + (j * 64 + lane) * 4;
-        float* p1 = l_red + DV * 256 + (j * 64 + lane) * 4;
+        float* p1 = p0 + LD;
+        float* p2 = p0 + 2 * LD;
+        float* p3 = p0 + 3 * LD;
         st4(p0, w == 0 ? S_t.v[j] : ld4(p0) + S_t.v[j]);
         st4(p1, w == 0 ? S_i.v[j] : ld4(p1) + S_i.v[j]);
+        st4(p2, w == 0 ? U_t.v[j] : ld4(p2) + U_t.v[j]);
+        st4(p3, w == 0 ? U_i.v[j] : ld4(p3) + U_i.v[j]);
+      }
+      if (lane == 0) {
+        float* s4 = l_red + 4 * LD;
+        s4[0] = (w == 0 ? 0.f : s4[0]) + sg_tt;
+        s4[1] = (w == 0 ? 0.f : s4[1]) + sg_ti;
+        s4[2] = (w == 0 ? 0.f : s4[2]) + sg_it;
+        s4[3] = (w == 0 ? 0.f : s4[3]) + sg_ii;
       }
     }
   }
   __syncthreads();
-  float* out = a.s2_part + (b * a.chunks + blockIdx.x) * (int64_t)(2 * D);
-  for (int i = threadIdx.x; i < 2 * D4; i += 256) {
+  const int64_t chunk = b * a.chunks + blockIdx.x;
+  float* out = a.s2_part + chunk * (int64_t)(2 * D);
+  float* out1 = a.s1_part + chunk * (int64_t)(2 * D + 4);
+  for (int i = threadIdx.x; i < 4 * D4; i += 256) {
     const int which = i / D4, c4 = i - which * D4;
-    st4(out + which * D + c4 * 4, ld4(l_red + which * DV * 256 + c4 * 4));
-  }
+    const float4 v = ld4(l_red + which * LD + c4 * 4);
+    st4((which < 2 ? out + which * D : out1 + (which - 2) * D) + c4 * 4, v);
+  }
+  if (threadIdx.x < 4) out1[2 * D + threadIdx.x] = l_red[4 * LD + threadIdx.x];
 }
 
 int launch_pair_layer1(const PairArgs& a, hipStream_t st) {
@@ -509,6 +453,63 @@
   return DRIN_OK;
 }
 
+__global__ void __launch_bounds__(256) k_mention_layer1(const float* __restrict__ part, const float* __restrict__ hb_t,
+                                                        const float* __restrict__ hb_i, const float* __restrict__ hm, int ldhm,
+                                                        const float* __restrict__ b_h1, const float* __restrict__ u_img,
+                                                        float* __restrict__ out, int B, int D, int chunks, float inv_n) {
+  const int64_t b = blockIdx.y;
+  const int d = blockIdx.x * 256 + threadIdx.x;
+  if (d >= D) return;
+  float ut = 0.f, ui = 0.f, s_tt = 0.f, s_ti = 0.f, s_it = 0.f, s_ii = 0.f;
+  for (int c = 0; c < chunks; ++c) {
+    const float* p = part + (b * chunks + c) * (int64_t)(2 * D + 4);
+    ut += p[d];
+    ui += p[D + d];
+    s_tt += p[2 * D];
+    s_ti += p[2 * D + 1];
+    s_it += p[2 * D + 2];
+    s_ii += p[2 * D + 3];
+  }
+  if (u_img) {
+    ut += u_img[b * D + d];
+    ui += u_img[((int64_t)B + b) * D + d];
+  }
+  const float ht = hb_t[d], hi = hb_i[d], bh = b_h1[d];
+  out[b * D + d] = ((ut + s_tt * ht) + s_ti * hi) * inv_n + (hm[b * ldhm + d] + bh);
+  out[((int64_t)B + b) * D + d] = ((ui + s_it * ht) + s_ii * hi) * inv_n + (hm[((int64_t)B + b) * ldhm + d] + bh);
+}
+
+int launch_mention_layer1(const float* part, const float* hb_t, const float* hb_i, const float* hm, int ldhm, const float* b_h1,
+                          const float* u_img, float* out, int B, int D, int N, int chunks, hipStream_t st) {
+  if (B <= 0) return DRIN_OK;
+  KernelTimer timer(DRIN_KC_GCN, st);
+  hipLaunchKernelGGL(k_mention_layer1, dim3((unsigned)cdiv(D, 256), (unsigned)B), dim3(256), 0, st, part, hb_t, hb_i, hm, ldhm,
+                     b_h1, u_img, out, B, D, chunks, 1.0f / (float)N);
+  DRIN_CHECK_LAUNCH("k_mention_layer1");
+  return DRIN_OK;
+}
+
+__global__ void __launch_bounds__(256) k_sum_image_partials(const float* __restrict__ part, float* __restrict__ s_img, int B, int R,
+                                                            int chunks) {
+  const int64_t b = blockIdx.y;
+  const int i = (blockIdx.x * 256 + threadIdx.x) * 4;
+  if (i >= 2 * R) return;
+  const float* src = part + (b * chunks) * (int64_t)(2 * R) + i;
+  float4 s = make_float4(0.f, 0.f, 0.f, 0.f);
+  for (int c = 0; c < chunks; ++c) s = s + ld4(src + (int64_t)c * (2 * R));
+  const int which = i >= R;
+  st4(s_img + ((int64_t)which * B + b) * R + (i - which * R), s);
+}
+
+int launch_sum_image_partials(const float* part, float* s_img, int B, int R, int chunks, hipStream_t st) {
+  if (B <= 0) return DRIN_OK;
+  KernelTimer timer(DRIN_KC_GCN, st);
+  hipLaunchKernelGGL(k_sum_image_partials, dim3((unsigned)cdiv(2 * R / 4, 256), (unsigned)B), dim3(256), 0, st, part, s_img, B, R,
+                     chunks);
+  DRIN_CHECK_LAUNCH("k_sum_image_partials");
+  return DRIN_OK;
+}
+
 __global__ void __launch_bounds__(256) k_mention_input2(const float* __restrict__ part, const float* __restrict__ mt1,
                                                         float* __restrict__ out, int D, int chunks, float inv_n) {
   const int64_t b = blockIdx.y;
```

Result: no change. 28.53 million pairs/s (median of 5 runs) (+0.7%).
